# hyx1999/SAM-Decoding

Hardware: AMD Instinct MI355X
Metric: tokens/sec (+ mean accepted tokens), Vicuna-7B bs=1, samd_sam_only draft+verify (higher is better)
Workload: dtype f16

## Files before the change

### sam-decoding_amd/csrc/gemm_kernels.hip

```cpp
#include <hip/hip_runtime.h>
#include <cstdlib>
#include "samd_common.h"

#define LAUNCHCHK() do { hipError_t e_ = hipGetLastError(); if (e_ != hipSuccess) { samd_set_error("kernel launch: %s", hipGetErrorString(e_)); return SAMD_E_HIP; } } while (0)

static int samd_cu_count() { return samd_device_cus(); }

typedef _Float16 half8 __attribute__((ext_vector_type(8)));
typedef __bf16 bf16x8 __attribute__((ext_vector_type(8)));
typedef float floatx4 __attribute__((ext_vector_type(4)));
typedef unsigned u32x4 __attribute__((ext_vector_type(4)));

struct GF16 { typedef _Float16 elem; typedef half8 vec8;
    static __device__ __forceinline__ floatx4 mfma(half8 a, half8 b, floatx4 c) { return __builtin_amdgcn_mfma_f32_16x16x32_f16(a, b, c, 0, 0, 0); } };
struct GBF16 { typedef __bf16 elem; typedef bf16x8 vec8;
    static __device__ __forceinline__ floatx4 mfma(bf16x8 a, bf16x8 b, floatx4 c) { return __builtin_amdgcn_mfma_f32_16x16x32_bf16(a, b, c, 0, 0, 0); } };

#define GEMM_KC 256
#define GEMM_WAVES 8
#define GEMM_COLS (16 * GEMM_WAVES)

typedef __attribute__((address_space(1))) const void *gptr_t;
typedef __attribute__((address_space(3))) void *lptr_t;

#ifdef SAMD_GEMM_ABLATE
__device__ int samd_abl_flag;
#endif

template <typename TT, int RT, int EPI, int DEPTH, bool GM = false>
__global__ __launch_bounds__(64 * GEMM_WAVES, RT >= 3 || DEPTH > 2 ? 2 : GEMM_WAVES / 2) void k_gemm_skinny(const typename TT::elem *__restrict__ A, const typename TT::elem *__restrict__ W,
                                                        float *__restrict__ partial, typename TT::elem *__restrict__ out,
                                                        int K, int N, int n_chunks, int n_splits) {
    typedef typename TT::elem E;
    typedef typename TT::vec8 V8;
    constexpr int R = 16 * RT;
    constexpr int NT = 64 * GEMM_WAVES;
    constexpr int XV = (R * 32) / NT;
    constexpr int NB = DEPTH + 1;
    extern __shared__ __attribute__((aligned(1024))) char gemm_lds[];
    E (*xs)[R][GEMM_KC] = reinterpret_cast<E (*)[R][GEMM_KC]>(gemm_lds);

    const int tid = threadIdx.x, w = tid >> 6, l = tid & 63, n = l & 15, g = l >> 4;
    const int n0 = blockIdx.x * GEMM_COLS + 16 * w;
    const int split = blockIdx.y;
    const int c0 = (int)((long long)split * n_chunks / n_splits), c1 = (int)((long long)(split + 1) * n_chunks / n_splits);
    constexpr size_t WCH = GM ? 8192 : 65536, WU = GM ? 1024 : 8192;
    const int ws = GM ? __builtin_amdgcn_readfirstlane(GEMM_WAVES * (int)blockIdx.x + w) : (int)blockIdx.x;
    const char *wtile = reinterpret_cast<const char *>(W) + (size_t)ws * n_chunks * WCH;
    const uint32_t wlane = (uint32_t)(GM ? l : tid) * 16;
    const uint32_t lds_base = (uint32_t)(uintptr_t)(lptr_t)&xs[0][0][0];

    floatx4 acc[RT];
#pragma unroll
    for (int mt = 0; mt < RT; mt++) acc[mt] = (floatx4){0.f, 0.f, 0.f, 0.f};

    u32x4 wr[DEPTH][4][2];
    auto load_wb = [&](u32x4 (&dst)[4][2], int c, int b) {
        const char *p = wtile + (size_t)c * WCH;
#pragma unroll
        for (int j = 0; j < 2; j++)
            asm volatile("global_load_dwordx4 %0, %1, %2 nt" : "=v"(dst[b][j]) : "v"(wlane), "s"(p + WU * (2 * b + j)) : "memory");
    };
    auto stage_xi = [&](int c, int buf, int i) {
        const int slot = tid + NT * i, row = slot >> 5, pos = slot & 31, unit = pos ^ (row & 15);
        const E *src = A + (size_t)row * K + (size_t)c * GEMM_KC + 8 * unit;
        E *dst = &xs[buf][0][0] + (size_t)(NT * i + 64 * w) * 8;
        __builtin_amdgcn_global_load_lds((gptr_t)src, (lptr_t)dst, 16, 0, 0);
        asm volatile("" ::: "memory");
    };
    auto load_w = [&](u32x4 (&dst)[4][2], int c) {
#pragma unroll
        for (int b = 0; b < 4; b++) load_wb(dst, c, b);
    };
    auto stage_x = [&](int c, int buf) {
#pragma unroll
        for (int i = 0; i < XV; i++) stage_xi(c, buf, i);
    };
    auto landed = [&](int younger_in_flight) {
        if (DEPTH > 2 && younger_in_flight >= 2) asm volatile("s_waitcnt vmcnt(%0)" : : "n"(2 * (8 + XV)) : "memory");
        else if (younger_in_flight >= 1) asm volatile("s_waitcnt vmcnt(%0)" : : "n"(8 + XV) : "memory");
        else asm volatile("s_waitcnt vmcnt(0)" : : : "memory");
        __builtin_amdgcn_s_barrier();
        asm volatile("" ::: "memory");
    };
    auto phase = [&](u32x4 (&cur)[4][2], int c, int buf) {
        landed(c1 - 1 - c);
        const uint32_t xbase = lds_base + (uint32_t)buf * (R * GEMM_KC * 2) + (uint32_t)n * (GEMM_KC * 2);
#pragma unroll
        for (int b = 0; b < 4; b++) {
            const uint32_t u0 = (uint32_t)((8 * b + 2 * g) ^ n) * 16, u1 = (uint32_t)((8 * b + 2 * g + 1) ^ n) * 16;
            const uint32_t a0 = xbase + u0, a1 = xbase + u1;
            u32x4 r[RT][2];
            if constexpr (RT == 1)
                asm volatile("ds_read_b128 %0, %2\n\tds_read_b128 %1, %3\n\ts_waitcnt lgkmcnt(0)" : "=&v"(r[0][0]), "=&v"(r[0][1]) : "v"(a0), "v"(a1));
            else if constexpr (RT == 2)
                asm volatile("ds_read_b128 %0, %4\n\tds_read_b128 %1, %5\n\tds_read_b128 %2, %4 offset:8192\n\tds_read_b128 %3, %5 offset:8192\n\t"
                             "s_waitcnt lgkmcnt(0)" : "=&v"(r[0][0]), "=&v"(r[0][1]), "=&v"(r[1][0]), "=&v"(r[1][1]) : "v"(a0), "v"(a1));
            else if constexpr (RT == 3)
                asm volatile("ds_read_b128 %0, %6\n\tds_read_b128 %1, %7\n\tds_read_b128 %2, %6 offset:8192\n\tds_read_b128 %3, %7 offset:8192\n\t"
                             "ds_read_b128 %4, %6 offset:16384\n\tds_read_b128 %5, %7 offset:16384\n\ts_waitcnt lgkmcnt(0)"
                             : "=&v"(r[0][0]), "=&v"(r[0][1]), "=&v"(r[1][0]), "=&v"(r[1][1]), "=&v"(r[2][0]), "=&v"(r[2][1]) : "v"(a0), "v"(a1));
            else
                asm volatile("ds_read_b128 %0, %8\n\tds_read_b128 %1, %9\n\tds_read_b128 %2, %8 offset:8192\n\tds_read_b128 %3, %9 offset:8192\n\t"
                             "ds_read_b128 %4, %8 offset:16384\n\tds_read_b128 %5, %9 offset:16384\n\tds_read_b128 %6, %8 offset:24576\n\t"
                             "ds_read_b128 %7, %9 offset:24576\n\ts_waitcnt lgkmcnt(0)"
                             : "=&v"(r[0][0]), "=&v"(r[0][1]), "=&v"(r[1][0]), "=&v"(r[1][1]), "=&v"(r[2][0]), "=&v"(r[2][1]), "=&v"(r[3][0]), "=&v"(r[3][1])
                             : "v"(a0), "v"(a1));
#pragma unroll
            for (int mt = 0; mt < RT; mt++) {
                acc[mt] = TT::mfma(__builtin_bit_cast(V8, r[mt][0]), __builtin_bit_cast(V8, cur[b][0]), acc[mt]);
                acc[mt] = TT::mfma(__builtin_bit_cast(V8, r[mt][1]), __builtin_bit_cast(V8, cur[b][1]), acc[mt]);
            }
            if (RT >= 3 && c + DEPTH < c1) {
                load_wb(cur, c + DEPTH, b);
                if (b < XV) stage_xi(c + DEPTH, buf == 0 ? NB - 1 : buf - 1, b);
            }
        }
        if (RT < 3 && c + DEPTH < c1) { load_w(cur, c + DEPTH); stage_x(c + DEPTH, buf == 0 ? NB - 1 : buf - 1); }
    };
    if (c0 < c1) {
#pragma unroll
        for (int d = 0; d < DEPTH; d++)
            if (c0 + d < c1) { load_w(wr[d], c0 + d); stage_x(c0 + d, d); }
        int buf = 0;
        for (int c = c0; c < c1; c += DEPTH) {
#pragma unroll
            for (int d = 0; d < DEPTH; d++)
                if (c + d < c1) { phase(wr[d], c + d, buf); buf = buf == NB - 1 ? 0 : buf + 1; }
        }
    }
    if constexpr (EPI == 1) {
        float *ex = reinterpret_cast<float *>(gemm_lds);
        __syncthreads();
        if (w >= 4) {
#pragma unroll
            for (int mt = 0; mt < RT; mt++)
#pragma unroll
                for (int r = 0; r < 4; r++) ex[(16 * mt + 4 * g + r) * 64 + 16 * (w - 4) + n] = acc[mt][r];
        }
        __syncthreads();
        if (w < 4) {
#pragma unroll
            for (int mt = 0; mt < RT; mt++)
#pragma unroll
                for (int r = 0; r < 4; r++) {
                    const int m = 16 * mt + 4 * g + r;
                    const float gf = (float)(E)acc[mt][r], uf = (float)(E)ex[m * 64 + 16 * w + n];
                    const E sv = (E)(gf / (1.f + __expf(-gf)));
                    out[(size_t)m * (N / 2) + blockIdx.x * 64 + 16 * w + n] = (E)((float)sv * uf);
                }
        }
        return;
    }
#pragma unroll
    for (int mt = 0; mt < RT; mt++) {
#pragma unroll
        for (int r = 0; r < 4; r++) {
            const int m = 16 * mt + 4 * g + r;
            if (out) out[(size_t)m * N + n0 + n] = (E)acc[mt][r];
            else __hip_atomic_store(&partial[((size_t)split * R + m) * N + n0 + n], acc[mt][r], __ATOMIC_RELAXED, __HIP_MEMORY_SCOPE_AGENT);
        }
    }
}

struct NormArgs { const float *ssq; const void *g; int tiles; float inv_hidden; float eps; };

#define NORM_NS 16
template <int NT>
__device__ __forceinline__ void norm_issue(const NormArgs &na, float (&sv)[NORM_NS]) {
    const int tid = threadIdx.x, row = tid & 15, p = tid >> 4;
#pragma unroll
    for (int k = 0; k < NORM_NS; k++) {
        sv[k] = 0.f;
        if ((NT / 16) * k >= na.tiles) continue;
        int t = p + (NT / 16) * k;
        t = t < na.tiles ? t : na.tiles - 1;
        const float *src = na.ssq + (size_t)t * 16 + row;
        asm volatile("global_load_dword %0, %1, off" : "=v"(sv[k]) : "v"(src) : "memory");
    }
}
template <int NT>
__device__ __forceinline__ void norm_finish(const NormArgs &na, float (&sv)[NORM_NS], float *part , float *rs ) {
    const int tid = threadIdx.x, row = tid & 15, p = tid >> 4;
    static_assert(NORM_NS == 16, "");
    asm volatile("" : "+v"(sv[0]), "+v"(sv[1]), "+v"(sv[2]), "+v"(sv[3]), "+v"(sv[4]), "+v"(sv[5]), "+v"(sv[6]), "+v"(sv[7]),
                      "+v"(sv[8]), "+v"(sv[9]), "+v"(sv[10]), "+v"(sv[11]), "+v"(sv[12]), "+v"(sv[13]), "+v"(sv[14]), "+v"(sv[15]) : : "memory");
    float s = 0.f;
#pragma unroll
    for (int k = 0; k < NORM_NS; k++) s += (p + (NT / 16) * k < na.tiles) ? sv[k] : 0.f;
    part[p * 16 + row] = s;
    asm volatile("s_waitcnt lgkmcnt(0)" ::: "memory");
    __builtin_amdgcn_s_barrier();
    asm volatile("" ::: "memory");
    if (tid < 16) {
        float tot = 0.f;
        for (int k = 0; k < NT / 16; k++) tot += part[k * 16 + tid];
        rs[tid] = rsqrtf(tot * na.inv_hidden + na.eps);
    }
    asm volatile("s_waitcnt lgkmcnt(0)" ::: "memory");
    __builtin_amdgcn_s_barrier();
    asm volatile("" ::: "memory");
}

template <typename E>
__device__ __forceinline__ u32x4 norm_scale8(u32x4 xraw, u32x4 graw, float rs) {
    const E *xe = reinterpret_cast<const E *>(&xraw);
    const E *ge = reinterpret_cast<const E *>(&graw);
    u32x4 out;
    E *oe = reinterpret_cast<E *>(&out);
#pragma unroll
    for (int j = 0; j < 8; j++) { const E h = (E)((float)xe[j] * rs); oe[j] = (E)((float)ge[j] * (float)h); }
    return out;
}


template <int DEPTH, int PC>
__device__ __forceinline__ void gemm_wait_younger(int younger) {
    if constexpr (PC == 0) asm volatile("s_waitcnt vmcnt(0)" : : : "memory");
    else {
        if (DEPTH > 3 && younger >= 3) asm volatile("s_waitcnt vmcnt(%0)" : : "n"(3 * PC) : "memory");
        else if (DEPTH > 2 && younger >= 2) asm volatile("s_waitcnt vmcnt(%0)" : : "n"(2 * PC) : "memory");
        else if (younger >= 1) asm volatile("s_waitcnt vmcnt(%0)" : : "n"(PC) : "memory");
        else asm volatile("s_waitcnt vmcnt(0)" : : : "memory");
    }
}

template <typename TT, int RT, int DEPTH, int CG, bool NORM, int AR = 16>
__global__ __launch_bounds__(64 * GEMM_WAVES, RT >= 3 || NORM ? 2 : GEMM_WAVES / 2) void k_gemm_qkv_rope(
        const typename TT::elem *__restrict__ A, const typename TT::elem *__restrict__ W, int K, int n_chunks,
        const float *__restrict__ cs, const int *__restrict__ d_L, const int *__restrict__ d_n,
        typename TT::elem *__restrict__ q_out, typename TT::elem *__restrict__ k_cache, typename TT::elem *__restrict__ v_cache,
        int H, int Hkv, long long max_len, NormArgs na, int v_t) {
    typedef typename TT::elem E;
    typedef typename TT::vec8 V8;
    constexpr int R = 16 * RT;
    constexpr int NT = 64 * GEMM_WAVES;
    constexpr int XV = (R * 32) / NT;
    constexpr int NB = DEPTH + 1;
    constexpr int WL = 4;
    constexpr int TW = 16 * CG, PP = 8 * CG;
    constexpr int CH = CG * 8192;
    extern __shared__ __attribute__((aligned(1024))) char gemm_lds[];
    E (*xs)[R][GEMM_KC] = reinterpret_cast<E (*)[R][GEMM_KC]>(gemm_lds);

    const int tid = threadIdx.x, w = tid >> 6, l = tid & 63, n = l & 15, g = l >> 4;
    const bool streams = CG == 4 || w < 2 * CG;
    static_assert(AR == 16 || (AR == 8 && NORM && RT == 1), "8 activation rows: the norm-fold kernels only");
    const bool stager = AR == 16 || w < GEMM_WAVES / 2;
    const int cg = CG == 4 ? (w & 3) : (streams ? w % CG : 0), kh = CG == 4 ? (w >> 2) : (streams ? w / CG : 0);
    const char *wtile = reinterpret_cast<const char *>(W) + (size_t)blockIdx.x * n_chunks * CH;
    const uint32_t wlane = (uint32_t)(64 * (CG * kh + cg) + l) * 16;
    const uint32_t lds_base = (uint32_t)(uintptr_t)(lptr_t)&xs[0][0][0];
    const int n_rows = d_n[0], L = d_L[0];

    floatx4 acc[RT];
#pragma unroll
    for (int mt = 0; mt < RT; mt++) acc[mt] = (floatx4){0.f, 0.f, 0.f, 0.f};

    u32x4 wr[DEPTH][2][2];
    auto load_wb = [&](u32x4 (&dst)[2][2], int c, int bl) {
        const char *p = wtile + (size_t)c * CH;
#pragma unroll
        for (int j = 0; j < 2; j++)
            asm volatile("global_load_dwordx4 %0, %1, %2 nt" : "=v"(dst[bl][j]) : "v"(wlane), "s"(p + (CH / 4) * (2 * bl + j)) : "memory");
    };
    static_assert(!NORM || RT == 1, "the norm-fold path is built for the 16-row tile");
    constexpr int XL = NORM ? 2 * XV : XV;
    u32x4 xr[NORM ? DEPTH : 1][NORM ? XV : 1], gr[NORM ? DEPTH : 1][NORM ? XV : 1];
    __shared__ float norm_part[NORM ? (NT / 16) * 16 : 1], norm_rs[NORM ? 16 : 1];
    auto stage_xi = [&](int c, int buf, int i, int d) {
        const int slot = tid + NT * i, row = slot >> 5, pos = slot & 31, unit = pos ^ (row & 15);
        const E *src = A + (size_t)row * K + (size_t)c * GEMM_KC + 8 * unit;
        if constexpr (NORM) {
            const E *gsrc = reinterpret_cast<const E *>(na.g) + (size_t)c * GEMM_KC + 8 * unit;
            asm volatile("global_load_dwordx4 %0, %1, off" : "=v"(xr[d][i]) : "v"(src) : "memory");
            asm volatile("global_load_dwordx4 %0, %1, off" : "=v"(gr[d][i]) : "v"(gsrc) : "memory");
        } else {
            E *dst = &xs[buf][0][0] + (size_t)(NT * i + 64 * w) * 8;
            __builtin_amdgcn_global_load_lds((gptr_t)src, (lptr_t)dst, 16, 0, 0);
            asm volatile("" ::: "memory");
        }
    };
    auto issue = [&](u32x4 (&dst)[2][2], int c, int buf, int d) {
        if (streams) { load_wb(dst, c, 0); load_wb(dst, c, 1); }
        if (stager) {
#pragma unroll
            for (int i = 0; i < XV; i++) stage_xi(c, buf, i, d);
        }
    };
    auto scale_to_lds = [&](int buf, int d) {
        if constexpr (NORM) {
            if (!stager) return;
#pragma unroll
            for (int i = 0; i < XV; i++) {
                const int slot = tid + NT * i, row = slot >> 5;
                asm volatile("" : "+v"(xr[d][i]), "+v"(gr[d][i]) : : "memory");
                const u32x4 v = norm_scale8<E>(xr[d][i], gr[d][i], norm_rs[row]);
                *reinterpret_cast<u32x4 *>(&xs[buf][0][0] + (size_t)slot * 8) = v;
            }
        }
    };
    auto landed = [&](int younger, int buf, int d) {
        if (streams) { if (stager) gemm_wait_younger<DEPTH, WL + XL>(younger); else gemm_wait_younger<DEPTH, WL>(younger); }
        else { if (stager) gemm_wait_younger<DEPTH, XL>(younger); else gemm_wait_younger<DEPTH, 0>(younger); }
        if constexpr (NORM) { scale_to_lds(buf, d); asm volatile("s_waitcnt lgkmcnt(0)" ::: "memory"); }
        __builtin_amdgcn_s_barrier();
        asm volatile("" ::: "memory");
    };
    auto phase = [&](u32x4 (&cur)[2][2], int c, int buf, int d) {
        landed(n_chunks - 1 - c, buf, d);
        const uint32_t xbase = lds_base + (uint32_t)buf * (R * GEMM_KC * 2) + (uint32_t)n * (GEMM_KC * 2);
#pragma unroll
        for (int bl = 0; bl < 2; bl++) {
            if (!streams) break;
            const int b = 2 * kh + bl;
            const uint32_t a0 = xbase + (uint32_t)((8 * b + 2 * g) ^ n) * 16, a1 = xbase + (uint32_t)((8 * b + 2 * g + 1) ^ n) * 16;
            u32x4 r[RT][2];
            if constexpr (RT == 1)
                asm volatile("ds_read_b128 %0, %2\n\tds_read_b128 %1, %3\n\ts_waitcnt lgkmcnt(0)" : "=&v"(r[0][0]), "=&v"(r[0][1]) : "v"(a0), "v"(a1));
            else if constexpr (RT == 2)
                asm volatile("ds_read_b128 %0, %4\n\tds_read_b128 %1, %5\n\tds_read_b128 %2, %4 offset:8192\n\tds_read_b128 %3, %5 offset:8192\n\t"
                             "s_waitcnt lgkmcnt(0)" : "=&v"(r[0][0]), "=&v"(r[0][1]), "=&v"(r[1][0]), "=&v"(r[1][1]) : "v"(a0), "v"(a1));
            else if constexpr (RT == 3)
                asm volatile("ds_read_b128 %0, %6\n\tds_read_b128 %1, %7\n\tds_read_b128 %2, %6 offset:8192\n\tds_read_b128 %3, %7 offset:8192\n\t"
                             "ds_read_b128 %4, %6 offset:16384\n\tds_read_b128 %5, %7 offset:16384\n\ts_waitcnt lgkmcnt(0)"
                             : "=&v"(r[0][0]), "=&v"(r[0][1]), "=&v"(r[1][0]), "=&v"(r[1][1]), "=&v"(r[2][0]), "=&v"(r[2][1]) : "v"(a0), "v"(a1));
            else
                asm volatile("ds_read_b128 %0, %8\n\tds_read_b128 %1, %9\n\tds_read_b128 %2, %8 offset:8192\n\tds_read_b128 %3, %9 offset:8192\n\t"
                             "ds_read_b128 %4, %8 offset:16384\n\tds_read_b128 %5, %9 offset:16384\n\tds_read_b128 %6, %8 offset:24576\n\t"
                             "ds_read_b128 %7, %9 offset:24576\n\ts_waitcnt lgkmcnt(0)"
                             : "=&v"(r[0][0]), "=&v"(r[0][1]), "=&v"(r[1][0]), "=&v"(r[1][1]), "=&v"(r[2][0]), "=&v"(r[2][1]), "=&v"(r[3][0]), "=&v"(r[3][1])
                             : "v"(a0), "v"(a1));
#pragma unroll
            for (int mt = 0; mt < RT; mt++) {
                acc[mt] = TT::mfma(__builtin_bit_cast(V8, r[mt][0]), __builtin_bit_cast(V8, cur[bl][0]), acc[mt]);
                acc[mt] = TT::mfma(__builtin_bit_cast(V8, r[mt][1]), __builtin_bit_cast(V8, cur[bl][1]), acc[mt]);
            }
        }
        if (c + DEPTH < n_chunks) issue(cur, c + DEPTH, buf == 0 ? NB - 1 : buf - 1, d);
    };
    float norm_sv[NORM ? NORM_NS : 1];
    if constexpr (NORM) norm_issue<NT>(na, norm_sv);
#pragma unroll
    for (int d = 0; d < DEPTH; d++)
        if (d < n_chunks) issue(wr[d], d, d, d);
    if constexpr (AR == 8) {
        if (!stager) {
#pragma unroll
            for (int bz = 0; bz < NB; bz++) *reinterpret_cast<u32x4 *>(&xs[bz][0][0] + (size_t)tid * 8) = (u32x4){0u, 0u, 0u, 0u};
        }
    }
    if constexpr (NORM) {
        if (n_chunks >= DEPTH) {
            if (streams) { if (stager) asm volatile("s_waitcnt vmcnt(%0)" : : "n"(DEPTH * (WL + XL)) : "memory"); else asm volatile("s_waitcnt vmcnt(%0)" : : "n"(DEPTH * WL) : "memory"); }
            else { if (stager) asm volatile("s_waitcnt vmcnt(%0)" : : "n"(DEPTH * XL) : "memory"); else asm volatile("s_waitcnt vmcnt(0)" : : : "memory"); }
        } else asm volatile("s_waitcnt vmcnt(0)" : : : "memory");
        norm_finish<NT>(na, norm_sv, norm_part, norm_rs);
    }
    {
        int buf = 0;
        for (int c = 0; c < n_chunks; c += DEPTH) {
#pragma unroll
            for (int d = 0; d < DEPTH; d++)
                if (c + d < n_chunks) { phase(wr[d], c + d, buf, d); buf = buf == NB - 1 ? 0 : buf + 1; }
        }
    }
    float *ex = reinterpret_cast<float *>(gemm_lds);
    __syncthreads();
    if (streams) {
#pragma unroll
        for (int mt = 0; mt < RT; mt++)
#pragma unroll
            for (int r = 0; r < 4; r++) ex[(kh * R + 16 * mt + 4 * g + r) * TW + 16 * cg + n] = acc[mt][r];
    }
    __syncthreads();
    const bool vt_tile = v_t && ((PP * (int)blockIdx.x) >> 6) >= H + Hkv;
    for (int i = tid; i < R * PP; i += NT) {
        const int row = vt_tile ? i % R : i / PP, p = vt_tile ? i / R : i % PP;
        if (row >= n_rows || L + row >= max_len) continue;
        const float x1 = (float)(E)(ex[row * TW + p] + ex[(R + row) * TW + p]);
        const float x2 = (float)(E)(ex[row * TW + PP + p] + ex[(R + row) * TW + PP + p]);
        const int pair = PP * (int)blockIdx.x + p, head = pair >> 6, j = pair & 63;
        if (head >= H + Hkv) {
            if (v_t) {
                E *dst = v_cache + (size_t)(head - H - Hkv) * max_len * 128 + L + row;
                dst[(size_t)j * max_len] = (E)x1; dst[(size_t)(j + 64) * max_len] = (E)x2;
                continue;
            }
            E *dst = v_cache + ((size_t)(head - H - Hkv) * max_len + L + row) * 128;
            dst[j] = (E)x1; dst[j + 64] = (E)x2;
            continue;
        }
        const float c = cs[(size_t)row * 128 + j], sn = cs[(size_t)row * 128 + 64 + j];
        const E o1 = (E)(x1 * c - x2 * sn), o2 = (E)(x2 * c + x1 * sn);
        E *dst = head < H ? q_out + ((size_t)row * H + head) * 128 : k_cache + ((size_t)(head - H) * max_len + L + row) * 128;
        dst[j] = o1; dst[j + 64] = o2;
    }
}

template <int CG>
__global__ __launch_bounds__(256) void k_gemm_pack_qkv(const uint4 *__restrict__ W, uint4 *__restrict__ out, int N, int K) {
    const long long u = (long long)blockIdx.x * 256 + threadIdx.x;
    const long long total = (long long)N * K / 8;
    if (u >= total) return;
    constexpr int PP = 8 * CG;
    const int n_chunks = K / GEMM_KC;
    const long long blk = u / (512 * CG);
    const int in = (int)(u % (512 * CG)), jj = in / (128 * CG), x = in % (128 * CG), w = x >> 6, g = (x >> 4) & 3, n = x & 15, cg = w % CG, kh = w / CG;
    const int t = (int)(blk / n_chunks), c = (int)(blk % n_chunks), bl = jj >> 1, j = jj & 1;
    const int q = 16 * cg + n, pair = PP * t + (q < PP ? q : q - PP);
    const long long row = 128LL * (pair >> 6) + (pair & 63) + (q < PP ? 0 : 64), col = 256LL * c + 64 * (2 * kh + bl) + 16 * g + 8 * j;
    out[u] = W[(row * K + col) / 8];
}

static int qkv_tile_groups(int n_heads_total) {
    static const int env = [] { const char *e = getenv("SAMD_QKV_TILE"); return e ? atoi(e) : 0; }();
    const int n_cu = samd_cu_count();
    const int N = n_heads_total * 128;
    if (N % 48 != 0 || env == 64) return 4;
    if (env == 48) return 3;
    const int t48 = N / 48, t64 = N / 64;
    return ((t48 + n_cu - 1) / n_cu) * 48 < ((t64 + n_cu - 1) / n_cu) * 64 ? 3 : 4;
}

template <typename TT, int RT, int DEPTH, bool NORM, int AR = 16>
__global__ __launch_bounds__(64 * GEMM_WAVES, RT >= 3 || DEPTH > 2 ? 2 : GEMM_WAVES / 2) void k_gemm_pairs_silu(const typename TT::elem *__restrict__ A, const typename TT::elem *__restrict__ W,
                                                                                                     typename TT::elem *__restrict__ out, int K, int inter, int n_chunks, int n_pairs, NormArgs na) {
    typedef typename TT::elem E;
    typedef typename TT::vec8 V8;
    constexpr int R = 16 * RT;
    constexpr int NT = 64 * GEMM_WAVES;
    constexpr int XV = (R * 32) / NT;
    constexpr int NB = DEPTH + 1;
    extern __shared__ __attribute__((aligned(1024))) char gemm_lds[];
    E (*xs)[R][GEMM_KC] = reinterpret_cast<E (*)[R][GEMM_KC]>(gemm_lds);

    const int tid = threadIdx.x, w = __builtin_amdgcn_readfirstlane(tid >> 6), l = tid & 63, n = l & 15, g = l >> 4;
#ifdef SAMD_GEMM_ABLATE
    const int abl = samd_abl_flag;
#else
    constexpr int abl = 0;
#endif
    const int p0 = (int)((long long)blockIdx.x * n_pairs / gridDim.x), p1 = (int)((long long)(blockIdx.x + 1) * n_pairs / gridDim.x);
    const bool active = w < 2 * (p1 - p0);
    static_assert(AR == 16 || (AR == 8 && NORM && RT == 1), "8 activation rows: the norm-fold kernels only");
    const bool stager = AR == 16 || w < GEMM_WAVES / 2;
    const int gi = 2 * p0 + w;
    const char *wgrp = reinterpret_cast<const char *>(W) + (size_t)(active ? gi : 0) * n_chunks * 8192;
    const uint32_t wlane = (uint32_t)l * 16;
    const uint32_t lds_base = (uint32_t)(uintptr_t)(lptr_t)&xs[0][0][0];

    floatx4 acc[RT];
#pragma unroll
    for (int mt = 0; mt < RT; mt++) acc[mt] = (floatx4){0.f, 0.f, 0.f, 0.f};
    u32x4 wr[DEPTH][4][2];
    auto load_w = [&](u32x4 (&dst)[4][2], int c) {
        const char *p = wgrp + (size_t)c * 8192;
#pragma unroll
        for (int b = 0; b < 4; b++)
#pragma unroll
            for (int j = 0; j < 2; j++)
                asm volatile("global_load_dwordx4 %0, %1, %2 nt" : "=v"(dst[b][j]) : "v"(wlane), "s"(p + 1024 * (2 * b + j)) : "memory");
    };
    static_assert(!NORM || RT == 1, "the norm-fold path is built for the 16-row tile");
    constexpr int XL = NORM ? 2 * XV : XV;
    u32x4 xr[NORM ? DEPTH : 1][NORM ? XV : 1], gr[NORM ? DEPTH : 1][NORM ? XV : 1];
    __shared__ float norm_part[NORM ? (NT / 16) * 16 : 1], norm_rs[NORM ? 16 : 1];
    auto stage_x = [&](int c, int buf, int d) {
        if (!stager || (abl & 4)) return;
#pragma unroll
        for (int i = 0; i < XV; i++) {
            const int slot = tid + NT * i, row = slot >> 5, pos = slot & 31, unit = pos ^ (row & 15);
            const E *src = A + (size_t)((abl & 8) ? (row & 15) : row) * K + (size_t)c * GEMM_KC + 8 * unit;
            if constexpr (NORM) {
                const E *gsrc = reinterpret_cast<const E *>(na.g) + (size_t)c * GEMM_KC + 8 * unit;
                asm volatile("global_load_dwordx4 %0, %1, off" : "=v"(xr[d][i]) : "v"(src) : "memory");
                asm volatile("global_load_dwordx4 %0, %1, off" : "=v"(gr[d][i]) : "v"(gsrc) : "memory");
            } else {
                E *dst = &xs[buf][0][0] + (size_t)(NT * i + 64 * w) * 8;
                __builtin_amdgcn_global_load_lds((gptr_t)src, (lptr_t)dst, 16, 0, 0);
                asm volatile("" ::: "memory");
            }
        }
    };
    auto landed = [&](int younger, int buf, int d) {
        const bool stg = stager && !(abl & 4);
        if (active) { if (stg) gemm_wait_younger<DEPTH, 8 + XL>(younger); else gemm_wait_younger<DEPTH, 8>(younger); }
        else { if (stg) gemm_wait_younger<DEPTH, XL>(younger); else gemm_wait_younger<DEPTH, 0>(younger); }
        if constexpr (NORM) {
            if (stager) {
#pragma unroll
                for (int i = 0; i < XV; i++) {
                    const int slot = tid + NT * i, row = slot >> 5;
                    asm volatile("" : "+v"(xr[d][i]), "+v"(gr[d][i]) : : "memory");
                    const u32x4 v = norm_scale8<E>(xr[d][i], gr[d][i], norm_rs[row]);
                    *reinterpret_cast<u32x4 *>(&xs[buf][0][0] + (size_t)slot * 8) = v;
                }
            }
            asm volatile("s_waitcnt lgkmcnt(0)" ::: "memory");
        }
        if (!(abl & 1)) __builtin_amdgcn_s_barrier();
        asm volatile("" ::: "memory");
    };
    auto phase = [&](u32x4 (&cur)[4][2], int c, int buf, int d) {
        landed(n_chunks - 1 - c, buf, d);
        if (active && !(abl & 2)) {
            const uint32_t xbase = lds_base + (uint32_t)buf * (R * GEMM_KC * 2) + (uint32_t)n * (GEMM_KC * 2);
#pragma unroll
            for (int b = 0; b < 4; b++) {
                const uint32_t a0 = xbase + (uint32_t)((8 * b + 2 * g) ^ n) * 16, a1 = xbase + (uint32_t)((8 * b + 2 * g + 1) ^ n) * 16;
                u32x4 r[RT][2];
                if constexpr (RT == 1)
                    asm volatile("ds_read_b128 %0, %2\n\tds_read_b128 %1, %3\n\ts_waitcnt lgkmcnt(0)" : "=&v"(r[0][0]), "=&v"(r[0][1]) : "v"(a0), "v"(a1));
                else if constexpr (RT == 2)
                    asm volatile("ds_read_b128 %0, %4\n\tds_read_b128 %1, %5\n\tds_read_b128 %2, %4 offset:8192\n\tds_read_b128 %3, %5 offset:8192\n\t"
                                 "s_waitcnt lgkmcnt(0)" : "=&v"(r[0][0]), "=&v"(r[0][1]), "=&v"(r[1][0]), "=&v"(r[1][1]) : "v"(a0), "v"(a1));
                else if constexpr (RT == 3)
                    asm volatile("ds_read_b128 %0, %6\n\tds_read_b128 %1, %7\n\tds_read_b128 %2, %6 offset:8192\n\tds_read_b128 %3, %7 offset:8192\n\t"
                                 "ds_read_b128 %4, %6 offset:16384\n\tds_read_b128 %5, %7 offset:16384\n\ts_waitcnt lgkmcnt(0)"
                                 : "=&v"(r[0][0]), "=&v"(r[0][1]), "=&v"(r[1][0]), "=&v"(r[1][1]), "=&v"(r[2][0]), "=&v"(r[2][1]) : "v"(a0), "v"(a1));
                else
                    asm volatile("ds_read_b128 %0, %8\n\tds_read_b128 %1, %9\n\tds_read_b128 %2, %8 offset:8192\n\tds_read_b128 %3, %9 offset:8192\n\t"
                                 "ds_read_b128 %4, %8 offset:16384\n\tds_read_b128 %5, %9 offset:16384\n\tds_read_b128 %6, %8 offset:24576\n\t"
                                 "ds_read_b128 %7, %9 offset:24576\n\ts_waitcnt lgkmcnt(0)"
                                 : "=&v"(r[0][0]), "=&v"(r[0][1]), "=&v"(r[1][0]), "=&v"(r[1][1]), "=&v"(r[2][0]), "=&v"(r[2][1]), "=&v"(r[3][0]), "=&v"(r[3][1])
                                 : "v"(a0), "v"(a1));
#pragma unroll
                for (int mt = 0; mt < RT; mt++) {
                    acc[mt] = TT::mfma(__builtin_bit_cast(V8, r[mt][0]), __builtin_bit_cast(V8, cur[b][0]), acc[mt]);
                    acc[mt] = TT::mfma(__builtin_bit_cast(V8, r[mt][1]), __builtin_bit_cast(V8, cur[b][1]), acc[mt]);
                }
            }
        }
        if (c + DEPTH < n_chunks) { if (active) load_w(cur, c + DEPTH); stage_x(c + DEPTH, buf == 0 ? NB - 1 : buf - 1, d); }
    };
    float norm_sv[NORM ? NORM_NS : 1];
    if constexpr (NORM) norm_issue<NT>(na, norm_sv);
#pragma unroll
    for (int d = 0; d < DEPTH; d++)
        if (d < n_chunks) { if (active) load_w(wr[d], d); stage_x(d, d, d); }
    if constexpr (AR == 8) {
        if (!stager) {
#pragma unroll
            for (int bz = 0; bz < NB; bz++) *reinterpret_cast<u32x4 *>(&xs[bz][0][0] + (size_t)tid * 8) = (u32x4){0u, 0u, 0u, 0u};
        }
    }
    if constexpr (NORM) {
        if (n_chunks >= DEPTH) {
            if (active) { if (stager) asm volatile("s_waitcnt vmcnt(%0)" : : "n"(DEPTH * (8 + XL)) : "memory"); else asm volatile("s_waitcnt vmcnt(%0)" : : "n"(DEPTH * 8) : "memory"); }
            else { if (stager) asm volatile("s_waitcnt vmcnt(%0)" : : "n"(DEPTH * XL) : "memory"); else asm volatile("s_waitcnt vmcnt(0)" : : : "memory"); }
        } else asm volatile("s_waitcnt vmcnt(0)" : : : "memory");
        norm_finish<NT>(na, norm_sv, norm_part, norm_rs);
    }
    {
        int buf = 0;
        for (int c = 0; c < n_chunks; c += DEPTH) {
#pragma unroll
            for (int d = 0; d < DEPTH; d++)
                if (c + d < n_chunks) { phase(wr[d], c + d, buf, d); buf = buf == NB - 1 ? 0 : buf + 1; }
        }
    }
    float *ex = reinterpret_cast<float *>(gemm_lds);
    __syncthreads();
    if (active && (w & 1)) {
#pragma unroll
        for (int mt = 0; mt < RT; mt++)
#pragma unroll
            for (int r = 0; r < 4; r++) ex[((w >> 1) * R + 16 * mt + 4 * g + r) * 16 + n] = acc[mt][r];
    }
    __syncthreads();
    if (active && !(w & 1)) {
        const int col = 16 * (p0 + (w >> 1)) + n;
#pragma unroll
        for (int mt = 0; mt < RT; mt++)
#pragma unroll
            for (int r = 0; r < 4; r++) {
                const int m = 16 * mt + 4 * g + r;
                const float gf = (float)(E)acc[mt][r], uf = (float)(E)ex[((w >> 1) * R + m) * 16 + n];
                const E sv = (E)(gf / (1.f + __expf(-gf)));
                out[(size_t)m * inter + col] = (E)((float)sv * uf);
            }
    }
}

template <typename TT, int ROWS, bool EARLY = false>
__global__ __launch_bounds__(64 * GEMM_WAVES, 2) void k_gemm_cs_residual(const typename TT::elem *__restrict__ A, const typename TT::elem *__restrict__ W,
                                                                           typename TT::elem *__restrict__ x, float *__restrict__ ssq, int K, int N, int n_chunks,
                                                                           const int *__restrict__ counter = nullptr, int *__restrict__ epoch = nullptr,
                                                                           int arrivals = 0) {
    typedef typename TT::elem E;
    typedef typename TT::vec8 V8;
    constexpr int CSD = 2;
    extern __shared__ __attribute__((aligned(1024))) char gemm_lds[];
    const int tid = threadIdx.x, w = __builtin_amdgcn_readfirstlane(tid >> 6), l = tid & 63, n = l & 15, g = l >> 4;
    E *xs = reinterpret_cast<E *>(gemm_lds) + (size_t)w * CSD * 16 * GEMM_KC;
    const uint32_t lds_base = (uint32_t)(uintptr_t)(lptr_t)xs;
    const char *wgrp = reinterpret_cast<const char *>(W) + (size_t)blockIdx.x * n_chunks * 8192;
    const uint32_t wlane = (uint32_t)l * 16;

    static_assert(ROWS == 8 || ROWS == 16, "");
    constexpr int AL = ROWS / 2;
    if constexpr (ROWS == 8) {
#pragma unroll
        for (int buf = 0; buf < CSD; buf++)
#pragma unroll
            for (int i = 4; i < 8; i++)
                *reinterpret_cast<u32x4 *>(xs + (size_t)buf * 16 * GEMM_KC + (size_t)(64 * i + l) * 8) = (u32x4){0u, 0u, 0u, 0u};
        asm volatile("s_waitcnt lgkmcnt(0)" ::: "memory");
    }
    floatx4 acc = (floatx4){0.f, 0.f, 0.f, 0.f};
    u32x4 wr[CSD][4][2];
    auto issue_w = [&](u32x4 (&dst)[4][2], int c) {
        const char *p = wgrp + (size_t)c * 8192;
#pragma unroll
        for (int b = 0; b < 4; b++)
#pragma unroll
            for (int j = 0; j < 2; j++)
                asm volatile("global_load_dwordx4 %0, %1, %2 nt" : "=v"(dst[b][j]) : "v"(wlane), "s"(p + 1024 * (2 * b + j)) : "memory");
    };
    auto issue_a = [&](int c, int buf) {
#pragma unroll
        for (int i = 0; i < AL; i++) {
            const int slot = l + 64 * i, row = slot >> 5, pos = slot & 31, unit = pos ^ (row & 15);
            const E *src = A + (size_t)row * K + (size_t)c * GEMM_KC + 8 * unit;
            E *dst_l = xs + (size_t)buf * 16 * GEMM_KC + (size_t)(64 * i) * 8;
            __builtin_amdgcn_global_load_lds((gptr_t)src, (lptr_t)dst_l, 16, 0, 0);
            asm volatile("" ::: "memory");
        }
    };
    auto issue = [&](u32x4 (&dst)[4][2], int c, int buf) { issue_w(dst, c); issue_a(c, buf); };
    auto phase = [&](u32x4 (&cur)[4][2], int c, int buf, bool more) {
        if (more) { if constexpr (EARLY) asm volatile("s_waitcnt vmcnt(%0)" : : "n"(AL) : "memory"); else asm volatile("s_waitcnt vmcnt(%0)" : : "n"(8 + AL) : "memory"); }
        else asm volatile("s_waitcnt vmcnt(0)" ::: "memory");
        const uint32_t xbase = lds_base + (uint32_t)buf * (16 * GEMM_KC * 2) + (uint32_t)n * (GEMM_KC * 2);
#pragma unroll
        for (int b = 0; b < 4; b++) {
            const uint32_t a0 = xbase + (uint32_t)((8 * b + 2 * g) ^ n) * 16, a1 = xbase + (uint32_t)((8 * b + 2 * g + 1) ^ n) * 16;
            u32x4 r0, r1;
            asm volatile("ds_read_b128 %0, %2\n\tds_read_b128 %1, %3\n\ts_waitcnt lgkmcnt(0)" : "=&v"(r0), "=&v"(r1) : "v"(a0), "v"(a1));
            acc = TT::mfma(__builtin_bit_cast(V8, r0), __builtin_bit_cast(V8, cur[b][0]), acc);
            acc = TT::mfma(__builtin_bit_cast(V8, r1), __builtin_bit_cast(V8, cur[b][1]), acc);
        }
    };
    const int mine = (n_chunks - w + GEMM_WAVES - 1) / GEMM_WAVES;
    if constexpr (EARLY) {
        if (mine > 0) issue_w(wr[0], w);
        if (mine > 1) issue_w(wr[1], w + GEMM_WAVES);
        __shared__ int my_epoch;
        if (tid == 0) {
            const int e = epoch[blockIdx.x];
            const int target = (e + 1) * arrivals;
            for (int spin = 0; spin < (1 << 22); spin++) {
                if (__hip_atomic_load(counter, __ATOMIC_RELAXED, __HIP_MEMORY_SCOPE_AGENT) >= target) break;
                __builtin_amdgcn_s_sleep(4);
            }
            my_epoch = e;
        }
        __syncthreads();
        __builtin_amdgcn_fence(__ATOMIC_ACQUIRE, "agent");
        if (mine > 0) issue_a(w, 0);
        if (mine > 1) issue_a(w + GEMM_WAVES, 1);
        if (mine > 0) phase(wr[0], w, 0, mine > 1);
        if (mine > 1) phase(wr[1], w + GEMM_WAVES, 1, false);
        if (tid == 0) epoch[blockIdx.x] = my_epoch + 1;
    } else {
        if (mine > 0) issue(wr[0], w, 0);
        if (mine > 1) issue(wr[1], w + GEMM_WAVES, 1);
        for (int i = 0; i < mine; i += 2) {
            phase(wr[0], w + GEMM_WAVES * i, 0, i + 1 < mine);
            if (i + 2 < mine) issue(wr[0], w + GEMM_WAVES * (i + 2), 0);
            if (i + 1 < mine) {
                phase(wr[1], w + GEMM_WAVES * (i + 1), 1, i + 2 < mine);
                if (i + 3 < mine) issue(wr[1], w + GEMM_WAVES * (i + 3), 1);
            }
        }
    }
    __syncthreads();
    float *ex = reinterpret_cast<float *>(gemm_lds);
#pragma unroll
    for (int r = 0; r < 4; r++) ex[(w * 16 + 4 * g + r) * 16 + n] = acc[r];
    __syncthreads();
    if (tid < 16 * ROWS) {
        const int row = tid >> 4, col = tid & 15;
        float sum = 0.f;
#pragma unroll
        for (int k = 0; k < GEMM_WAVES; k++) sum += ex[(k * 16 + row) * 16 + col];
        E *xp = x + (size_t)row * N + 16 * blockIdx.x + col;
        const E o = (E)sum;
        const E y = (E)((float)*xp + (float)o);
        *xp = y;
        float q = (float)y * (float)y;
        q += __shfl_xor(q, 1); q += __shfl_xor(q, 2); q += __shfl_xor(q, 4); q += __shfl_xor(q, 8);
        if (col == 0) ssq[(size_t)blockIdx.x * 16 + row] = q;
    }
}

__global__ __launch_bounds__(256) void k_gemm_pack_groups(const uint4 *__restrict__ W, uint4 *__restrict__ out, int N, int K) {
    const long long u = (long long)blockIdx.x * 256 + threadIdx.x;
    const long long total = (long long)N * K / 8;
    if (u >= total) return;
    const int n_chunks = K / GEMM_KC;
    const long long blk = u >> 9;
    const int in = (int)(u & 511), jj = in >> 6, lane = in & 63, g = lane >> 4, n = lane & 15, b = jj >> 1, j = jj & 1;
    const long long gi = blk / n_chunks; const int c = (int)(blk % n_chunks);
    const long long row = 16 * gi + n, col = 256LL * c + 64 * b + 16 * g + 8 * j;
    out[u] = W[(row * K + col) / 8];
}

__global__ __launch_bounds__(256) void k_gemm_pack(const uint4 *__restrict__ W, uint4 *__restrict__ out, int N, int K) {
    const long long u = (long long)blockIdx.x * 256 + threadIdx.x;
    const long long total = (long long)N * K / 8;
    if (u >= total) return;
    const int n_chunks = K / GEMM_KC;
    const long long blk = u >> 12;
    const int in = (int)(u & 4095), jj = in >> 9, tid = in & 511, w = tid >> 6, g = (tid >> 4) & 3, n = tid & 15;
    const int t = (int)(blk / n_chunks), c = (int)(blk % n_chunks), b = jj >> 1, j = jj & 1;
    const long long row = 128LL * t + 16 * w + n, col = 256LL * c + 64 * b + 16 * g + 8 * j;
    out[u] = W[(row * K + col) / 8];
}

template <typename TT, int RT, int EPI, int DEPTH, bool GM = false>
static hipError_t gemm_launch(dim3 grid, hipStream_t st, const void *A, const void *W, float *partial, void *out, int K, int N, int chunks, int splits) {
    constexpr int lds = (DEPTH + 1) * 16 * RT * GEMM_KC * 2;
    if constexpr (lds > 65536) {
        static unsigned long long done = 0ull;
        const hipError_t attr = samd_reserve_lds((const void *)k_gemm_skinny<TT, RT, EPI, DEPTH, GM>, lds, &done);
        if (attr != hipSuccess) return attr;
    }
    hipLaunchKernelGGL((k_gemm_skinny<TT, RT, EPI, DEPTH, GM>), grid, dim3(64 * GEMM_WAVES), lds, st, (const typename TT::elem *)A, (const typename TT::elem *)W, partial,
                       (typename TT::elem *)out, K, N, chunks, splits);
    return hipSuccess;
}

template <int EPI, bool GM = false>
static hipError_t gemm_dispatch(int dtype, int rows_pad, dim3 grid, hipStream_t st, const void *A, const void *W, float *partial, void *out, int K, int N, int chunks,
                                int splits) {
#define GO(TT, RT, D) return gemm_launch<TT, RT, EPI, D, GM>(grid, st, A, W, partial, out, K, N, chunks, splits)
#define ROWS(TT) do { if (rows_pad == 16) GO(TT, 1, 2); else if (rows_pad == 32) GO(TT, 2, 2); else if (rows_pad == 48) GO(TT, 3, 2); else GO(TT, 4, 2); } while (0)
    if (dtype == SAMD_F16) ROWS(GF16); else ROWS(GBF16);
#undef ROWS
#undef GO
}

template <typename TT, int RT, int DEPTH, int CG, bool NORM = false, int AR = 16>
static hipError_t qkv_rope_launch(hipStream_t st, const void *A, const void *W, int K, int tiles, const float *cs, const int *d_L, const int *d_n, void *q, void *k, void *v,
                                  int H, int Hkv, long long max_len, int v_t, NormArgs na = NormArgs{nullptr, nullptr, 0, 0.f, 0.f}) {
    constexpr int lds_a = (DEPTH + 1) * 16 * RT * GEMM_KC * 2, lds_e = 2 * 16 * RT * 16 * CG * 4, lds = lds_a > lds_e ? lds_a : lds_e;
    if constexpr (lds > 60000) {
        static unsigned long long done = 0ull;
        const hipError_t attr = samd_reserve_lds((const void *)k_gemm_qkv_rope<TT, RT, DEPTH, CG, NORM, AR>, lds + 4096, &done);
        if (attr != hipSuccess) return attr;
    }
    hipLaunchKernelGGL((k_gemm_qkv_rope<TT, RT, DEPTH, CG, NORM, AR>), dim3(tiles), dim3(64 * GEMM_WAVES), lds, st, (const typename TT::elem *)A, (const typename TT::elem *)W, K, K / GEMM_KC,
                       cs, d_L, d_n, (typename TT::elem *)q, (typename TT::elem *)k, (typename TT::elem *)v, H, Hkv, max_len, na, v_t);
    return hipSuccess;
}

template <typename TT, int RT, int DEPTH, bool NORM = false, int AR = 16>
static hipError_t pairs_silu_launch(hipStream_t st, int grid, const void *A, const void *W, void *out, int K, int inter, int n_pairs,
                                    NormArgs na = NormArgs{nullptr, nullptr, 0, 0.f, 0.f}) {
    constexpr int lds_a = (DEPTH + 1) * 16 * RT * GEMM_KC * 2, lds_e = 4 * 16 * RT * 16 * 4, lds = lds_a > lds_e ? lds_a : lds_e;
    if constexpr (lds > 60000) {
        static unsigned long long done = 0ull;
        const hipError_t attr = samd_reserve_lds((const void *)k_gemm_pairs_silu<TT, RT, DEPTH, NORM, AR>, lds + 4096, &done);
        if (attr != hipSuccess) return attr;
    }
    hipLaunchKernelGGL((k_gemm_pairs_silu<TT, RT, DEPTH, NORM, AR>), dim3(grid), dim3(64 * GEMM_WAVES), lds, st, (const typename TT::elem *)A, (const typename TT::elem *)W,
                       (typename TT::elem *)out, K, inter, K / GEMM_KC, n_pairs, na);
    return hipSuccess;
}

extern "C" {

int samd_gemm_splits(int32_t N, int32_t K, int32_t rows_pad) {
    static const int env_cap = [] { const char *e = getenv("SAMD_GEMM_SPLIT_CAP"); const int v = e ? atoi(e) : 8; return v < 1 ? 1 : (v > 8 ? 8 : v); }();
    static const int env_fixed = [] { const char *e = getenv("SAMD_GEMM_SPLITS"); const int v = e ? atoi(e) : 0; return v < 0 ? 0 : (v > 8 ? 8 : v); }();
    const int cols = N / GEMM_COLS, chunks = K / GEMM_KC;
    (void)rows_pad;
    if (env_fixed) return env_fixed > chunks ? (chunks < 1 ? 1 : chunks) : env_fixed;
    int s = 256 / (cols > 0 ? cols : 1);
    if (s > env_cap) s = env_cap;
    if (s > chunks) s = chunks;
    return s < 1 ? 1 : s;
}

int64_t samd_gemm_workspace(int32_t rows_pad, int32_t N, int32_t splits) { return (int64_t)splits * rows_pad * N * 4; }

int samd_gemm_skinny_silu(const void *d_A, const void *d_W, int32_t rows_pad, int32_t N, int32_t K, void *d_out, int32_t dtype, void *stream) {
    if (!d_A || !d_W || !d_out || (rows_pad != 16 && rows_pad != 32 && rows_pad != 48 && rows_pad != 64) || N < GEMM_COLS || N % GEMM_COLS != 0 || K < GEMM_KC ||
        K % GEMM_KC != 0 || (dtype != SAMD_F16 && dtype != SAMD_BF16)) {
        samd_set_error("samd_gemm_skinny_silu: unsupported shape (rows 16/32/48/64, N %% 128 == 0, K %% 256 == 0) or null pointer"); return SAMD_E_INVALID;
    }
    const hipError_t e = gemm_dispatch<1>(dtype, rows_pad, dim3(N / GEMM_COLS, 1), (hipStream_t)stream, d_A, d_W, nullptr, d_out, K, N, K / GEMM_KC, 1);
    if (e != hipSuccess) { samd_set_error("samd_gemm_skinny_silu: %s", hipGetErrorString(e)); return SAMD_E_HIP; }
    LAUNCHCHK();
    return SAMD_OK;
}

int samd_gemm_pack_weights(const void *d_W, void *d_packed, int32_t N, int32_t K, void *stream) {
    if (!d_W || !d_packed || d_W == d_packed || N < GEMM_COLS || N % GEMM_COLS != 0 || K < GEMM_KC || K % GEMM_KC != 0) {
        samd_set_error("samd_gemm_pack_weights: needs N %% 128 == 0, K %% 256 == 0 and distinct buffers"); return SAMD_E_INVALID;
    }
    const long long units = (long long)N * K / 8;
    hipLaunchKernelGGL(k_gemm_pack, dim3((unsigned)((units + 255) / 256)), dim3(256), 0, (hipStream_t)stream, (const uint4 *)d_W, (uint4 *)d_packed, N, K);
    LAUNCHCHK();
    return SAMD_OK;
}

int samd_gemm_pack_groups(const void *d_W, void *d_packed, int32_t N, int32_t K, void *stream) {
    if (!d_W || !d_packed || d_W == d_packed || N < 16 || N % 16 != 0 || K < GEMM_KC || K % GEMM_KC != 0) {
        samd_set_error("samd_gemm_pack_groups: needs N %% 16 == 0, K %% 256 == 0 and distinct buffers"); return SAMD_E_INVALID;
    }
    const long long units = (long long)N * K / 8;
    hipLaunchKernelGGL(k_gemm_pack_groups, dim3((unsigned)((units + 255) / 256)), dim3(256), 0, (hipStream_t)stream, (const uint4 *)d_W, (uint4 *)d_packed, N, K);
    LAUNCHCHK();
    return SAMD_OK;
}

int samd_gemm_pairs_silu_norm(const void *d_x, const float *d_ssq, const void *d_norm_weight, float eps, const void *d_Wg, int32_t rows_pad, int32_t inter, int32_t K,
                              void *d_out, int32_t dtype, void *stream) {
    if (!d_x || !d_ssq || !d_norm_weight || !d_Wg || !d_out || (rows_pad != 16 && rows_pad != 8) || inter < 16 || inter % 16 != 0 || K < GEMM_KC || K % GEMM_KC != 0 ||
        K / 16 > 32 * NORM_NS || (dtype != SAMD_F16 && dtype != SAMD_BF16)) {
        samd_set_error("samd_gemm_pairs_silu_norm: unsupported shape (8 or 16 rows, inter %% 16 == 0, K %% 256 == 0, K <= 8192, f16/bf16) or null pointer"); return SAMD_E_INVALID;
    }
    const int n_cu = samd_cu_count();
    const int n_pairs = inter / 16;
    int grid = n_pairs < n_cu ? n_pairs : n_cu;
    while ((n_pairs + grid - 1) / grid > 4) grid += n_cu;
    const NormArgs na{d_ssq, d_norm_weight, K / 16, 1.f / (float)K, eps};
    hipStream_t st = (hipStream_t)stream;
    const hipError_t e = rows_pad == 8
        ? (dtype == SAMD_F16 ? pairs_silu_launch<GF16, 1, 3, true, 8>(st, grid, d_x, d_Wg, d_out, K, inter, n_pairs, na)
                             : pairs_silu_launch<GBF16, 1, 3, true, 8>(st, grid, d_x, d_Wg, d_out, K, inter, n_pairs, na))
        : (dtype == SAMD_F16 ? pairs_silu_launch<GF16, 1, 3, true>(st, grid, d_x, d_Wg, d_out, K, inter, n_pairs, na)
                             : pairs_silu_launch<GBF16, 1, 3, true>(st, grid, d_x, d_Wg, d_out, K, inter, n_pairs, na));
    if (e != hipSuccess) { samd_set_error("samd_gemm_pairs_silu_norm: %s", hipGetErrorString(e)); return SAMD_E_HIP; }
    LAUNCHCHK();
    return SAMD_OK;
}

int samd_gemm_cs_residual(const void *d_A, const void *d_Wg, int32_t rows_pad, int32_t N, int32_t K, void *d_x, float *d_ssq, int32_t dtype, void *stream) {
    if (!d_A || !d_Wg || !d_x || !d_ssq || (rows_pad != 16 && rows_pad != 8) || N < 16 || N % 16 != 0 || K < GEMM_KC || K % GEMM_KC != 0 || (dtype != SAMD_F16 && dtype != SAMD_BF16)) {
        samd_set_error("samd_gemm_cs_residual: unsupported shape (8 or 16 rows, N %% 16 == 0, K %% 256 == 0, f16/bf16) or null pointer"); return SAMD_E_INVALID;
    }
    constexpr int lds = GEMM_WAVES * 2 * 16 * GEMM_KC * 2;
    hipStream_t st = (hipStream_t)stream;
    hipError_t e = hipSuccess;
#define GO(TT, ROWS, ET) do { static unsigned long long done = 0ull; \
        e = samd_reserve_lds((const void *)k_gemm_cs_residual<TT, ROWS>, lds, &done); \
        if (e == hipSuccess) hipLaunchKernelGGL((k_gemm_cs_residual<TT, ROWS>), dim3(N / 16), dim3(64 * GEMM_WAVES), lds, st, (const ET *)d_A, (const ET *)d_Wg, (ET *)d_x, d_ssq, K, N, K / GEMM_KC, (const int *)nullptr, (int *)nullptr, 0); } while (0)
    if (dtype == SAMD_F16) { if (rows_pad == 8) GO(GF16, 8, _Float16); else GO(GF16, 16, _Float16); }
    else { if (rows_pad == 8) GO(GBF16, 8, __bf16); else GO(GBF16, 16, __bf16); }
#undef GO
    if (e != hipSuccess) { samd_set_error("samd_gemm_cs_residual: %s", hipGetErrorString(e)); return SAMD_E_HIP; }
    LAUNCHCHK();
    return SAMD_OK;
}

int samd_gemm_cs_residual_early(const void *d_A, const void *d_Wg, int32_t N, int32_t K, void *d_x, float *d_ssq, int32_t dtype, const int32_t *d_counter,
                                int32_t *d_epoch, int32_t arrivals, void *stream) {
    if (!d_A || !d_Wg || !d_x || !d_ssq || !d_counter || !d_epoch || arrivals < 1 || N < 16 || N % 16 != 0 || K != 2 * GEMM_WAVES * GEMM_KC ||
        (dtype != SAMD_F16 && dtype != SAMD_BF16)) {
        samd_set_error("samd_gemm_cs_residual_early: unsupported shape (K must be 4096, N %% 16 == 0, f16/bf16) or null pointer"); return SAMD_E_INVALID;
    }
    constexpr int lds = GEMM_WAVES * 2 * 16 * GEMM_KC * 2;
    hipStream_t st = (hipStream_t)stream;
    hipError_t e = hipSuccess;
    if (dtype == SAMD_F16) {
        static unsigned long long done = 0ull;
        e = samd_reserve_lds((const void *)k_gemm_cs_residual<GF16, 8, true>, lds, &done);
        if (e == hipSuccess) hipLaunchKernelGGL((k_gemm_cs_residual<GF16, 8, true>), dim3(N / 16), dim3(64 * GEMM_WAVES), lds, st, (const _Float16 *)d_A, (const _Float16 *)d_Wg,
                                                (_Float16 *)d_x, d_ssq, K, N, K / GEMM_KC, d_counter, d_epoch, arrivals);
    } else {
        static unsigned long long done = 0ull;
        e = samd_reserve_lds((const void *)k_gemm_cs_residual<GBF16, 8, true>, lds, &done);
        if (e == hipSuccess) hipLaunchKernelGGL((k_gemm_cs_residual<GBF16, 8, true>), dim3(N / 16), dim3(64 * GEMM_WAVES), lds, st, (const __bf16 *)d_A, (const __bf16 *)d_Wg,
                                                (__bf16 *)d_x, d_ssq, K, N, K / GEMM_KC, d_counter, d_epoch, arrivals);
    }
    if (e != hipSuccess) { samd_set_error("samd_gemm_cs_residual_early: %s", hipGetErrorString(e)); return SAMD_E_HIP; }
    LAUNCHCHK();
    return SAMD_OK;
}

int samd_gemm_pairs_silu(const void *d_A, const void *d_Wg, int32_t rows_pad, int32_t inter, int32_t K, void *d_out, int32_t dtype, void *stream) {
    if (!d_A || !d_Wg || !d_out || (rows_pad != 16 && rows_pad != 32 && rows_pad != 48 && rows_pad != 64) || inter < 16 || inter % 16 != 0 || K < GEMM_KC ||
        K % GEMM_KC != 0 || (dtype != SAMD_F16 && dtype != SAMD_BF16)) {
        samd_set_error("samd_gemm_pairs_silu: unsupported shape (rows 16/32/48/64, inter %% 16 == 0, K %% 256 == 0, f16/bf16) or null pointer"); return SAMD_E_INVALID;
    }
    const int n_cu = samd_cu_count();
    const int n_pairs = inter / 16;
    int grid = n_pairs < n_cu ? n_pairs : n_cu;
    while ((n_pairs + grid - 1) / grid > 4) grid += n_cu;
    hipStream_t st = (hipStream_t)stream;
    hipError_t e;
    static const int depth_env = [] { const char *e = getenv("SAMD_PAIRS_DEPTH"); return e ? atoi(e) : 0; }();
#ifdef SAMD_GEMM_ABLATE
    static const int abl_set = [] { const char *e = getenv("SAMD_GEMM_ABL"); const int v = e ? atoi(e) : 0; return hipMemcpyToSymbol(HIP_SYMBOL(samd_abl_flag), &v, 4) == hipSuccess ? 1 : -1; }();
    (void)abl_set;
#endif
#define ARGS st, grid, d_A, d_Wg, d_out, K, inter, n_pairs
#define GO(TT) (rows_pad == 16 ? (depth_env == 2 ? pairs_silu_launch<TT, 1, 2>(ARGS) : depth_env == 4 ? pairs_silu_launch<TT, 1, 4>(ARGS) : pairs_silu_launch<TT, 1, 3>(ARGS)) \
                : rows_pad == 32 ? (depth_env == 2 ? pairs_silu_launch<TT, 2, 2>(ARGS) : pairs_silu_launch<TT, 2, 3>(ARGS)) \
                : rows_pad == 48 ? pairs_silu_launch<TT, 3, 2>(ARGS) : pairs_silu_launch<TT, 4, 2>(ARGS))
    e = dtype == SAMD_F16 ? GO(GF16) : GO(GBF16);
#undef GO
#undef ARGS
    if (e != hipSuccess) { samd_set_error("samd_gemm_pairs_silu: %s", hipGetErrorString(e)); return SAMD_E_HIP; }
    LAUNCHCHK();
    return SAMD_OK;
}

int samd_gemm_pack_qkv64(const void *d_W, void *d_packed, int32_t n_heads_total, int32_t K, void *stream) {
    if (!d_W || !d_packed || d_W == d_packed || n_heads_total < 1 || K < GEMM_KC || K % GEMM_KC != 0) {
        samd_set_error("samd_gemm_pack_qkv64: needs K %% 256 == 0, whole 128-column heads and distinct buffers"); return SAMD_E_INVALID;
    }
    const long long units = (long long)n_heads_total * 128 * K / 8;
    if (qkv_tile_groups(n_heads_total) == 3)
        hipLaunchKernelGGL(k_gemm_pack_qkv<3>, dim3((unsigned)((units + 255) / 256)), dim3(256), 0, (hipStream_t)stream, (const uint4 *)d_W, (uint4 *)d_packed, n_heads_total * 128, K);
    else
        hipLaunchKernelGGL(k_gemm_pack_qkv<4>, dim3((unsigned)((units + 255) / 256)), dim3(256), 0, (hipStream_t)stream, (const uint4 *)d_W, (uint4 *)d_packed, n_heads_total * 128, K);
    LAUNCHCHK();
    return SAMD_OK;
}

static int gemm_qkv_rope_impl(const void *d_A, const void *d_W64, int32_t rows_pad, int32_t K, const float *d_cs, const int32_t *d_cache_length, const int32_t *d_n,
                              void *d_q_out, void *d_k_cache, void *d_v_cache, int32_t n_heads, int32_t n_kv_heads, int32_t head_dim, int64_t max_len,
                              int32_t dtype, void *stream, int v_t) {
    if (!d_A || !d_W64 || !d_cs || !d_cache_length || !d_n || !d_q_out || !d_k_cache || !d_v_cache || head_dim != 128 || n_heads < 1 || n_kv_heads < 1 ||
        (rows_pad != 16 && rows_pad != 32 && rows_pad != 48 && rows_pad != 64) || K < GEMM_KC || K % GEMM_KC != 0 || (dtype != SAMD_F16 && dtype != SAMD_BF16)) {
        samd_set_error("samd_gemm_qkv_rope: unsupported shape (rows 16/32/48/64, head_dim 128, K %% 256 == 0, f16/bf16) or null pointer"); return SAMD_E_INVALID;
    }
    static const int depth_env = [] { const char *e = getenv("SAMD_QKV_DEPTH"); return e ? atoi(e) : 0; }();
    const int groups = qkv_tile_groups(n_heads + 2 * n_kv_heads);
    const int tiles = (n_heads + 2 * n_kv_heads) * 128 / (16 * groups);
    hipStream_t st = (hipStream_t)stream;
    hipError_t e = hipSuccess;
#define GO(TT, RT, D, CG) e = qkv_rope_launch<TT, RT, D, CG>(st, d_A, d_W64, K, tiles, d_cs, d_cache_length, d_n, d_q_out, d_k_cache, d_v_cache, n_heads, n_kv_heads, (long long)max_len, v_t)
#define ROWS(TT, CG) do { if (rows_pad == 16) { if (depth_env == 2) GO(TT, 1, 2, CG); else if (depth_env == 3) GO(TT, 1, 3, CG); else GO(TT, 1, 4, CG); } \
                          else if (rows_pad == 32) { if (depth_env == 2) GO(TT, 2, 2, CG); else GO(TT, 2, 4, CG); } \
                          else if (rows_pad == 48) GO(TT, 3, 3, CG); else GO(TT, 4, 3, CG); } while (0)
    if (groups == 3) { if (dtype == SAMD_F16) ROWS(GF16, 3); else ROWS(GBF16, 3); }
    else { if (dtype == SAMD_F16) ROWS(GF16, 4); else ROWS(GBF16, 4); }
#undef ROWS
#undef GO
    if (e != hipSuccess) { samd_set_error("samd_gemm_qkv_rope: %s", hipGetErrorString(e)); return SAMD_E_HIP; }
    LAUNCHCHK();
    return SAMD_OK;
}

int samd_gemm_qkv_rope(const void *d_A, const void *d_W64, int32_t rows_pad, int32_t K, const float *d_cs, const int32_t *d_cache_length, const int32_t *d_n,
                       void *d_q_out, void *d_k_cache, void *d_v_cache, int32_t n_heads, int32_t n_kv_heads, int32_t head_dim, int64_t max_len,
                       int32_t dtype, void *stream) {
    return gemm_qkv_rope_impl(d_A, d_W64, rows_pad, K, d_cs, d_cache_length, d_n, d_q_out, d_k_cache, d_v_cache, n_heads, n_kv_heads, head_dim, max_len, dtype, stream, 0);
}

int samd_gemm_qkv_rope_vt(const void *d_A, const void *d_W64, int32_t rows_pad, int32_t K, const float *d_cs, const int32_t *d_cache_length, const int32_t *d_n,
                          void *d_q_out, void *d_k_cache, void *d_vt_cache, int32_t n_heads, int32_t n_kv_heads, int32_t head_dim, int64_t max_len,
                          int32_t dtype, void *stream) {
    return gemm_qkv_rope_impl(d_A, d_W64, rows_pad, K, d_cs, d_cache_length, d_n, d_q_out, d_k_cache, d_vt_cache, n_heads, n_kv_heads, head_dim, max_len, dtype, stream, 1);
}

static int gemm_qkv_rope_norm_impl(const void *d_x, const float *d_ssq, const void *d_norm_weight, float eps, const void *d_W64, int32_t rows_pad, int32_t K,
                                   const float *d_cs, const int32_t *d_cache_length, const int32_t *d_n, void *d_q_out, void *d_k_cache, void *d_v_cache,
                                   int32_t n_heads, int32_t n_kv_heads, int32_t head_dim, int64_t max_len, int32_t dtype, void *stream, int v_t) {
    if (!d_x || !d_ssq || !d_norm_weight || !d_W64 || !d_cs || !d_cache_length || !d_n || !d_q_out || !d_k_cache || !d_v_cache || head_dim != 128 || n_heads < 1 ||
        n_kv_heads < 1 || (rows_pad != 16 && rows_pad != 8) || K < GEMM_KC || K % GEMM_KC != 0 || K / 16 > 32 * NORM_NS || (dtype != SAMD_F16 && dtype != SAMD_BF16)) {
        samd_set_error("samd_gemm_qkv_rope_norm: unsupported shape (8 or 16 rows, head_dim 128, K %% 256 == 0, K <= 8192, f16/bf16) or null pointer"); return SAMD_E_INVALID;
    }
    const int groups = qkv_tile_groups(n_heads + 2 * n_kv_heads);
    const int tiles = (n_heads + 2 * n_kv_heads) * 128 / (16 * groups);
    const NormArgs na{d_ssq, d_norm_weight, K / 16, 1.f / (float)K, eps};
    hipStream_t st = (hipStream_t)stream;
    hipError_t e = hipSuccess;
#define GO(TT, CG, AR) e = qkv_rope_launch<TT, 1, 4, CG, true, AR>(st, d_x, d_W64, K, tiles, d_cs, d_cache_length, d_n, d_q_out, d_k_cache, d_v_cache, n_heads, n_kv_heads, (long long)max_len, v_t, na)
    if (rows_pad == 8) {
        if (groups == 3) { if (dtype == SAMD_F16) GO(GF16, 3, 8); else GO(GBF16, 3, 8); }
        else { if (dtype == SAMD_F16) GO(GF16, 4, 8); else GO(GBF16, 4, 8); }
    } else {
        if (groups == 3) { if (dtype == SAMD_F16) GO(GF16, 3, 16); else GO(GBF16, 3, 16); }
        else { if (dtype == SAMD_F16) GO(GF16, 4, 16); else GO(GBF16, 4, 16); }
    }
#undef GO
    if (e != hipSuccess) { samd_set_error("samd_gemm_qkv_rope_norm: %s", hipGetErrorString(e)); return SAMD_E_HIP; }
    LAUNCHCHK();
    return SAMD_OK;
}

int samd_gemm_qkv_rope_norm(const void *d_x, const float *d_ssq, const void *d_norm_weight, float eps, const void *d_W64, int32_t rows_pad, int32_t K,
                            const float *d_cs, const int32_t *d_cache_length, const int32_t *d_n, void *d_q_out, void *d_k_cache, void *d_v_cache,
                            int32_t n_heads, int32_t n_kv_heads, int32_t head_dim, int64_t max_len, int32_t dtype, void *stream) {
    return gemm_qkv_rope_norm_impl(d_x, d_ssq, d_norm_weight, eps, d_W64, rows_pad, K, d_cs, d_cache_length, d_n, d_q_out, d_k_cache, d_v_cache, n_heads, n_kv_heads, head_dim,
                                   max_len, dtype, stream, 0);
}

int samd_gemm_qkv_rope_norm_vt(const void *d_x, const float *d_ssq, const void *d_norm_weight, float eps, const void *d_W64, int32_t rows_pad, int32_t K,
                               const float *d_cs, const int32_t *d_cache_length, const int32_t *d_n, void *d_q_out, void *d_k_cache, void *d_vt_cache,
                               int32_t n_heads, int32_t n_kv_heads, int32_t head_dim, int64_t max_len, int32_t dtype, void *stream) {
    return gemm_qkv_rope_norm_impl(d_x, d_ssq, d_norm_weight, eps, d_W64, rows_pad, K, d_cs, d_cache_length, d_n, d_q_out, d_k_cache, d_vt_cache, n_heads, n_kv_heads, head_dim,
                                   max_len, dtype, stream, 1);
}

int samd_gemm_skinny(const void *d_A, const void *d_W, int32_t rows_pad, int32_t N, int32_t K, int32_t splits, float *d_partial,
                     void *d_out, int32_t dtype, void *stream) {
    if (!d_A || !d_W || (rows_pad != 16 && rows_pad != 32 && rows_pad != 48 && rows_pad != 64) || N < GEMM_COLS || N % GEMM_COLS != 0 || K < GEMM_KC ||
        K % GEMM_KC != 0 || splits < 1 || splits > K / GEMM_KC || (splits == 1 ? !d_out : !d_partial) || (dtype != SAMD_F16 && dtype != SAMD_BF16)) {
        samd_set_error("samd_gemm_skinny: unsupported shape (rows 16/32/48/64, N %% 128 == 0, K %% 256 == 0) or null pointer"); return SAMD_E_INVALID;
    }
    const hipError_t e = gemm_dispatch<0>(dtype, rows_pad, dim3(N / GEMM_COLS, splits), (hipStream_t)stream, d_A, d_W, d_partial, splits == 1 ? d_out : nullptr, K, N,
                                          K / GEMM_KC, splits);
    if (e != hipSuccess) { samd_set_error("samd_gemm_skinny: %s", hipGetErrorString(e)); return SAMD_E_HIP; }
    LAUNCHCHK();
    return SAMD_OK;
}

int samd_gemm_skinny_groups(const void *d_A, const void *d_Wg, int32_t rows_pad, int32_t N, int32_t K, int32_t splits, float *d_partial,
                            void *d_out, int32_t dtype, void *stream) {
    if (!d_A || !d_Wg || (rows_pad != 16 && rows_pad != 32 && rows_pad != 48 && rows_pad != 64) || N < GEMM_COLS || N % GEMM_COLS != 0 || K < GEMM_KC ||
        K % GEMM_KC != 0 || splits < 1 || splits > K / GEMM_KC || (splits == 1 ? !d_out : !d_partial) || (dtype != SAMD_F16 && dtype != SAMD_BF16)) {
        samd_set_error("samd_gemm_skinny_groups: unsupported shape (rows 16/32/48/64, N %% 128 == 0, K %% 256 == 0) or null pointer"); return SAMD_E_INVALID;
    }
    const hipError_t e = gemm_dispatch<0, true>(dtype, rows_pad, dim3(N / GEMM_COLS, splits), (hipStream_t)stream, d_A, d_Wg, d_partial, splits == 1 ? d_out : nullptr, K, N,
                                                K / GEMM_KC, splits);
    if (e != hipSuccess) { samd_set_error("samd_gemm_skinny_groups: %s", hipGetErrorString(e)); return SAMD_E_HIP; }
    LAUNCHCHK();
    return SAMD_OK;
}

}

template <typename TT> struct F8Widen;
template <> struct F8Widen<GF16> {
    static __device__ __forceinline__ half8 cvt(unsigned w0, unsigned w1) {
        const auto a = __builtin_amdgcn_cvt_scalef32_pk_f16_fp8(w0, 1.0f, false), b = __builtin_amdgcn_cvt_scalef32_pk_f16_fp8(w0, 1.0f, true);
        const auto c = __builtin_amdgcn_cvt_scalef32_pk_f16_fp8(w1, 1.0f, false), d = __builtin_amdgcn_cvt_scalef32_pk_f16_fp8(w1, 1.0f, true);
        return __builtin_bit_cast(half8, (u32x4){__builtin_bit_cast(unsigned, a), __builtin_bit_cast(unsigned, b), __builtin_bit_cast(unsigned, c), __builtin_bit_cast(unsigned, d)});
    }
};
template <> struct F8Widen<GBF16> {
    static __device__ __forceinline__ bf16x8 cvt(unsigned w0, unsigned w1) {
        const auto a = __builtin_amdgcn_cvt_scalef32_pk_bf16_fp8(w0, 1.0f, false), b = __builtin_amdgcn_cvt_scalef32_pk_bf16_fp8(w0, 1.0f, true);
        const auto c = __builtin_amdgcn_cvt_scalef32_pk_bf16_fp8(w1, 1.0f, false), d = __builtin_amdgcn_cvt_scalef32_pk_bf16_fp8(w1, 1.0f, true);
        return __builtin_bit_cast(bf16x8, (u32x4){__builtin_bit_cast(unsigned, a), __builtin_bit_cast(unsigned, b), __builtin_bit_cast(unsigned, c), __builtin_bit_cast(unsigned, d)});
    }
};

template <typename TT, int RT, int DEPTH>
__global__ __launch_bounds__(64 * GEMM_WAVES, 2) void k_gemm_skinny_f8(const typename TT::elem *__restrict__ A, const unsigned char *__restrict__ W8,
                                                                     const float *__restrict__ scale, float *__restrict__ partial,
                                                                     typename TT::elem *__restrict__ out, int K, int N, int n_chunks, int n_splits) {
    typedef typename TT::elem E;
    constexpr int R = 16 * RT;
    constexpr int NT = 64 * GEMM_WAVES;
    constexpr int XV = (R * 32) / NT;
    constexpr int NB = DEPTH + 1;
    constexpr int PC = 4 + XV;
    constexpr size_t WCH = 32768, WU = 8192;
    extern __shared__ __attribute__((aligned(1024))) char gemm_lds[];
    E (*xs)[R][GEMM_KC] = reinterpret_cast<E (*)[R][GEMM_KC]>(gemm_lds);

    const int tid = threadIdx.x, w = tid >> 6, l = tid & 63, n = l & 15, g = l >> 4;
    const int n0 = blockIdx.x * GEMM_COLS + 16 * w;
    const int split = blockIdx.y;
    const int c0 = (int)((long long)split * n_chunks / n_splits), c1 = (int)((long long)(split + 1) * n_chunks / n_splits);
    const char *wtile = reinterpret_cast<const char *>(W8) + (size_t)blockIdx.x * n_chunks * WCH;
    const uint32_t wlane = (uint32_t)tid * 16;
    const uint32_t lds_base = (uint32_t)(uintptr_t)(lptr_t)&xs[0][0][0];
    const float sc = scale[n0 + n];

    floatx4 acc[RT];
#pragma unroll
    for (int mt = 0; mt < RT; mt++) acc[mt] = (floatx4){0.f, 0.f, 0.f, 0.f};

    u32x4 wr[DEPTH][4];
    auto load_wb = [&](u32x4 (&dst)[4], int c, int b) {
        const char *p = wtile + (size_t)c * WCH;
        asm volatile("global_load_dwordx4 %0, %1, %2 nt" : "=v"(dst[b]) : "v"(wlane), "s"(p + WU * b) : "memory");
    };
    auto stage_xi = [&](int c, int buf, int i) {
        const int slot = tid + NT * i, row = slot >> 5, pos = slot & 31, unit = pos ^ (row & 15);
        const E *src = A + (size_t)row * K + (size_t)c * GEMM_KC + 8 * unit;
        E *dst = &xs[buf][0][0] + (size_t)(NT * i + 64 * w) * 8;
        __builtin_amdgcn_global_load_lds((gptr_t)src, (lptr_t)dst, 16, 0, 0);
        asm volatile("" ::: "memory");
    };
    auto load_w = [&](u32x4 (&dst)[4], int c) {
#pragma unroll
        for (int b = 0; b < 4; b++) load_wb(dst, c, b);
    };
    auto stage_x = [&](int c, int buf) {
#pragma unroll
        for (int i = 0; i < XV; i++) stage_xi(c, buf, i);
    };
    auto phase = [&](u32x4 (&cur)[4], int c, int buf) {
        gemm_wait_younger<DEPTH, PC>(c1 - 1 - c);
        __builtin_amdgcn_s_barrier();
        asm volatile("" ::: "memory");
        const uint32_t xbase = lds_base + (uint32_t)buf * (R * GEMM_KC * 2) + (uint32_t)n * (GEMM_KC * 2);
#pragma unroll
        for (int b = 0; b < 4; b++) {
            const uint32_t a0 = xbase + (uint32_t)((8 * b + 2 * g) ^ n) * 16, a1 = xbase + (uint32_t)((8 * b + 2 * g + 1) ^ n) * 16;
            u32x4 r[RT][2];
            if constexpr (RT == 1)
                asm volatile("ds_read_b128 %0, %2\n\tds_read_b128 %1, %3\n\ts_waitcnt lgkmcnt(0)" : "=&v"(r[0][0]), "=&v"(r[0][1]) : "v"(a0), "v"(a1));
            else if constexpr (RT == 2)
                asm volatile("ds_read_b128 %0, %4\n\tds_read_b128 %1, %5\n\tds_read_b128 %2, %4 offset:8192\n\tds_read_b128 %3, %5 offset:8192\n\t"
                             "s_waitcnt lgkmcnt(0)" : "=&v"(r[0][0]), "=&v"(r[0][1]), "=&v"(r[1][0]), "=&v"(r[1][1]) : "v"(a0), "v"(a1));
            else if constexpr (RT == 3)
                asm volatile("ds_read_b128 %0, %6\n\tds_read_b128 %1, %7\n\tds_read_b128 %2, %6 offset:8192\n\tds_read_b128 %3, %7 offset:8192\n\t"
                             "ds_read_b128 %4, %6 offset:16384\n\tds_read_b128 %5, %7 offset:16384\n\ts_waitcnt lgkmcnt(0)"
                             : "=&v"(r[0][0]), "=&v"(r[0][1]), "=&v"(r[1][0]), "=&v"(r[1][1]), "=&v"(r[2][0]), "=&v"(r[2][1]) : "v"(a0), "v"(a1));
            else
                asm volatile("ds_read_b128 %0, %8\n\tds_read_b128 %1, %9\n\tds_read_b128 %2, %8 offset:8192\n\tds_read_b128 %3, %9 offset:8192\n\t"
                             "ds_read_b128 %4, %8 offset:16384\n\tds_read_b128 %5, %9 offset:16384\n\tds_read_b128 %6, %8 offset:24576\n\t"
                             "ds_read_b128 %7, %9 offset:24576\n\ts_waitcnt lgkmcnt(0)"
                             : "=&v"(r[0][0]), "=&v"(r[0][1]), "=&v"(r[1][0]), "=&v"(r[1][1]), "=&v"(r[2][0]), "=&v"(r[2][1]), "=&v"(r[3][0]), "=&v"(r[3][1])
                             : "v"(a0), "v"(a1));
            asm volatile("" : "+v"(cur[b]) : : "memory");
            const auto lo = F8Widen<TT>::cvt(cur[b][0], cur[b][1]), hi = F8Widen<TT>::cvt(cur[b][2], cur[b][3]);
#pragma unroll
            for (int mt = 0; mt < RT; mt++) {
                acc[mt] = TT::mfma(__builtin_bit_cast(typename TT::vec8, r[mt][0]), lo, acc[mt]);
                acc[mt] = TT::mfma(__builtin_bit_cast(typename TT::vec8, r[mt][1]), hi, acc[mt]);
            }
            if (RT >= 3 && c + DEPTH < c1) {
                load_wb(cur, c + DEPTH, b);
                if (b < XV) stage_xi(c + DEPTH, buf == 0 ? NB - 1 : buf - 1, b);
            }
        }
        if (RT < 3 && c + DEPTH < c1) { load_w(cur, c + DEPTH); stage_x(c + DEPTH, buf == 0 ? NB - 1 : buf - 1); }
    };
    if (c0 < c1) {
#pragma unroll
        for (int d = 0; d < DEPTH; d++)
            if (c0 + d < c1) { load_w(wr[d], c0 + d); stage_x(c0 + d, d); }
        int buf = 0;
        for (int c = c0; c < c1; c += DEPTH) {
#pragma unroll
            for (int d = 0; d < DEPTH; d++)
                if (c + d < c1) { phase(wr[d], c + d, buf); buf = buf == NB - 1 ? 0 : buf + 1; }
        }
    }
#pragma unroll
    for (int mt = 0; mt < RT; mt++) {
#pragma unroll
        for (int r = 0; r < 4; r++) {
            const int m = 16 * mt + 4 * g + r;
            const float v = acc[mt][r] * sc;
            if (out) out[(size_t)m * N + n0 + n] = (E)v;
            else __hip_atomic_store(&partial[((size_t)split * R + m) * N + n0 + n], v, __ATOMIC_RELAXED, __HIP_MEMORY_SCOPE_AGENT);
        }
    }
}

__global__ __launch_bounds__(256) void k_gemm_pack_f8(const uint4 *__restrict__ W8, uint4 *__restrict__ out, int N, int K) {
    const long long u = (long long)blockIdx.x * 256 + threadIdx.x;
    const long long total = (long long)N * K / 16;
    if (u >= total) return;
    const int n_chunks = K / GEMM_KC;
    const long long blk = u >> 11;
    const int in = (int)(u & 2047), b = in >> 9, tid = in & 511, w = tid >> 6, g = (tid >> 4) & 3, n = tid & 15;
    const int t = (int)(blk / n_chunks), c = (int)(blk % n_chunks);
    const long long row = 128LL * t + 16 * w + n, col = 256LL * c + 64 * b + 16 * g;
    out[u] = W8[(row * K + col) / 16];
}

template <typename TT, int RT, int DEPTH>
static hipError_t gemm_f8_launch(dim3 grid, hipStream_t st, const void *A, const void *W8, const float *scale, float *partial, void *out, int K, int N,
                                 int splits) {
    constexpr int lds = (DEPTH + 1) * 16 * RT * GEMM_KC * 2;
    if constexpr (lds > 65536) {
        static unsigned long long done = 0ull;
        const hipError_t attr = samd_reserve_lds((const void *)k_gemm_skinny_f8<TT, RT, DEPTH>, lds, &done);
        if (attr != hipSuccess) return attr;
    }
    hipLaunchKernelGGL((k_gemm_skinny_f8<TT, RT, DEPTH>), grid, dim3(64 * GEMM_WAVES), lds, st, (const typename TT::elem *)A, (const unsigned char *)W8, scale,
                       partial, (typename TT::elem *)out, K, N, K / GEMM_KC, splits);
    return hipSuccess;
}

extern "C" {

int samd_gemm_pack_f8(const void *d_W8, void *d_out, int32_t N, int32_t K, void *stream) {
    if (!d_W8 || !d_out || d_W8 == d_out || N < GEMM_COLS || N % GEMM_COLS != 0 || K < GEMM_KC || K % GEMM_KC != 0) {
        samd_set_error("samd_gemm_pack_f8: needs N %% 128 == 0, K %% 256 == 0 and distinct buffers"); return SAMD_E_INVALID;
    }
    const long long units = (long long)N * K / 16;
    hipLaunchKernelGGL(k_gemm_pack_f8, dim3((unsigned)((units + 255) / 256)), dim3(256), 0, (hipStream_t)stream, (const uint4 *)d_W8, (uint4 *)d_out, N, K);
    LAUNCHCHK();
    return SAMD_OK;
}

int samd_gemm_skinny_f8(const void *d_A, const void *d_W8p, const float *d_scale, int32_t rows_pad, int32_t N, int32_t K, int32_t splits, float *d_partial,
                        void *d_out, int32_t dtype, void *stream) {
    if (!d_A || !d_W8p || !d_scale || (rows_pad != 16 && rows_pad != 32 && rows_pad != 48 && rows_pad != 64) || N < GEMM_COLS || N % GEMM_COLS != 0 ||
        K < GEMM_KC || K % GEMM_KC != 0 || splits < 1 || splits > K / GEMM_KC || (splits == 1 ? !d_out : !d_partial) || (dtype != SAMD_F16 && dtype != SAMD_BF16)) {
        samd_set_error("samd_gemm_skinny_f8: unsupported shape (rows 16/32/48/64, N %% 128 == 0, K %% 256 == 0) or null pointer"); return SAMD_E_INVALID;
    }
    const dim3 grid(N / GEMM_COLS, splits);
    const hipStream_t st = (hipStream_t)stream;
    float *part = splits == 1 ? nullptr : d_partial;
    void *out = splits == 1 ? d_out : nullptr;
#define GO(TT, RT, D) e = gemm_f8_launch<TT, RT, D>(grid, st, d_A, d_W8p, d_scale, part, out, K, N, splits)
#define ROWS(TT) do { if (rows_pad == 16) GO(TT, 1, 4); else if (rows_pad == 32) GO(TT, 2, 4); else if (rows_pad == 48) GO(TT, 3, 4); else GO(TT, 4, 3); } while (0)
    hipError_t e;
    if (dtype == SAMD_F16) ROWS(GF16); else ROWS(GBF16);
#undef ROWS
#undef GO
    if (e != hipSuccess) { samd_set_error("samd_gemm_skinny_f8: %s", hipGetErrorString(e)); return SAMD_E_HIP; }
    LAUNCHCHK();
    return SAMD_OK;
}

}

template <typename TT> struct F4Widen;
template <> struct F4Widen<GF16> {
    static __device__ __forceinline__ half8 cvt(unsigned w, float s) {
        const auto a = __builtin_amdgcn_cvt_scalef32_pk_f16_fp4(w, s, 0), b = __builtin_amdgcn_cvt_scalef32_pk_f16_fp4(w, s, 1);
        const auto c = __builtin_amdgcn_cvt_scalef32_pk_f16_fp4(w, s, 2), d = __builtin_amdgcn_cvt_scalef32_pk_f16_fp4(w, s, 3);
        return __builtin_bit_cast(half8, (u32x4){__builtin_bit_cast(unsigned, a), __builtin_bit_cast(unsigned, b), __builtin_bit_cast(unsigned, c), __builtin_bit_cast(unsigned, d)});
    }
};
template <> struct F4Widen<GBF16> {
    static __device__ __forceinline__ bf16x8 cvt(unsigned w, float s) {
        const auto a = __builtin_amdgcn_cvt_scalef32_pk_bf16_fp4(w, s, 0), b = __builtin_amdgcn_cvt_scalef32_pk_bf16_fp4(w, s, 1);
        const auto c = __builtin_amdgcn_cvt_scalef32_pk_bf16_fp4(w, s, 2), d = __builtin_amdgcn_cvt_scalef32_pk_bf16_fp4(w, s, 3);
        return __builtin_bit_cast(bf16x8, (u32x4){__builtin_bit_cast(unsigned, a), __builtin_bit_cast(unsigned, b), __builtin_bit_cast(unsigned, c), __builtin_bit_cast(unsigned, d)});
    }
};

template <int DEPTH, int PC>
__device__ __forceinline__ void gemm_wait_younger_deep(int younger) {
    static_assert(DEPTH <= 8 && (DEPTH - 1) * PC <= 63, "vmcnt is a 6-bit counter");
#define SAMD_WAIT_IF(i) if (DEPTH > i && younger >= i) { asm volatile("s_waitcnt vmcnt(%0)" : : "n"(DEPTH > i ? i * PC : 0) : "memory"); return; }
    SAMD_WAIT_IF(7) SAMD_WAIT_IF(6) SAMD_WAIT_IF(5) SAMD_WAIT_IF(4) SAMD_WAIT_IF(3) SAMD_WAIT_IF(2) SAMD_WAIT_IF(1)
#undef SAMD_WAIT_IF
    asm volatile("s_waitcnt vmcnt(0)" : : : "memory");
}

template <int RT>
__device__ __forceinline__ void gemm_f4_read_a(u32x4 (&r)[RT][2], uint32_t a0, uint32_t a1) {
    if constexpr (RT == 1)
        asm volatile("ds_read_b128 %0, %2\n\tds_read_b128 %1, %3\n\ts_waitcnt lgkmcnt(0)" : "=&v"(r[0][0]), "=&v"(r[0][1]) : "v"(a0), "v"(a1));
    else if constexpr (RT == 2)
        asm volatile("ds_read_b128 %0, %4\n\tds_read_b128 %1, %5\n\tds_read_b128 %2, %4 offset:8192\n\tds_read_b128 %3, %5 offset:8192\n\t"
                     "s_waitcnt lgkmcnt(0)" : "=&v"(r[0][0]), "=&v"(r[0][1]), "=&v"(r[1][0]), "=&v"(r[1][1]) : "v"(a0), "v"(a1));
    else if constexpr (RT == 3)
        asm volatile("ds_read_b128 %0, %6\n\tds_read_b128 %1, %7\n\tds_read_b128 %2, %6 offset:8192\n\tds_read_b128 %3, %7 offset:8192\n\t"
                     "ds_read_b128 %4, %6 offset:16384\n\tds_read_b128 %5, %7 offset:16384\n\ts_waitcnt lgkmcnt(0)"
                     : "=&v"(r[0][0]), "=&v"(r[0][1]), "=&v"(r[1][0]), "=&v"(r[1][1]), "=&v"(r[2][0]), "=&v"(r[2][1]) : "v"(a0), "v"(a1));
    else
        asm volatile("ds_read_b128 %0, %8\n\tds_read_b128 %1, %9\n\tds_read_b128 %2, %8 offset:8192\n\tds_read_b128 %3, %9 offset:8192\n\t"
                     "ds_read_b128 %4, %8 offset:16384\n\tds_read_b128 %5, %9 offset:16384\n\tds_read_b128 %6, %8 offset:24576\n\t"
                     "ds_read_b128 %7, %9 offset:24576\n\ts_waitcnt lgkmcnt(0)"
                     : "=&v"(r[0][0]), "=&v"(r[0][1]), "=&v"(r[1][0]), "=&v"(r[1][1]), "=&v"(r[2][0]), "=&v"(r[2][1]), "=&v"(r[3][0]), "=&v"(r[3][1])
                     : "v"(a0), "v"(a1));
}

template <typename TT, int RT, int DEPTH>
__global__ __launch_bounds__(64 * GEMM_WAVES, 2) void k_gemm_skinny_f4(const typename TT::elem *__restrict__ A, const unsigned char *__restrict__ W4,
                                                                     float *__restrict__ partial, typename TT::elem *__restrict__ out, int K, int N,
                                                                     int n_chunks, int n_splits) {
    typedef typename TT::elem E;
    constexpr int R = 16 * RT;
    constexpr int NT = 64 * GEMM_WAVES;
    constexpr int XV = (R * 32) / NT;
    constexpr int NB = DEPTH + 1;
    constexpr int PC = 3 + XV;
    constexpr size_t WCH = 17408, WU = 8192, WS = 16384;
    extern __shared__ __attribute__((aligned(1024))) char gemm_lds[];
    E (*xs)[R][GEMM_KC] = reinterpret_cast<E (*)[R][GEMM_KC]>(gemm_lds);

    const int tid = threadIdx.x, w = tid >> 6, l = tid & 63, n = l & 15, g = l >> 4;
    const int n0 = blockIdx.x * GEMM_COLS + 16 * w;
    const int split = blockIdx.y;
    const int c0 = (int)((long long)split * n_chunks / n_splits), c1 = (int)((long long)(split + 1) * n_chunks / n_splits);
    const char *wtile = reinterpret_cast<const char *>(W4) + (size_t)blockIdx.x * n_chunks * WCH;
    const uint32_t wlane = (uint32_t)tid * 16, slane = (uint32_t)tid * 2;
    const uint32_t lds_base = (uint32_t)(uintptr_t)(lptr_t)&xs[0][0][0];

    floatx4 acc[RT];
#pragma unroll
    for (int mt = 0; mt < RT; mt++) acc[mt] = (floatx4){0.f, 0.f, 0.f, 0.f};

// ... 1261 lines not shown
```

### sam-decoding_amd/samd_hip/llama.py

```python
import ctypes as C
import math
import os

import torch

from . import (F16, BF16, MAX_DRAFT, TILE_ROWS, QkvEpilogue, SamdError, Session, Warm, _ptr, check, current_stream, lib, require_gpu,
               torch_dtype_code)
from . import fp8 as F8
from . import mxfp4 as MX
from . import int4 as I4
from . import moe as MOE


def _env_weight_format(weight_format):
    return weight_format if weight_format is not None else (os.environ.get("SAMD_WEIGHT_FORMAT") or None)


def _weight_format(weight_format, weights, dtype):
    has_f8 = any(l[k].dtype == torch.float8_e4m3fn for l in weights["layers"] for k in F8.PROJECTIONS if k in l)
    has_i4 = any(k + "_z" in l for l in weights["layers"] for k in I4.PROJECTIONS)
    has_f4 = any(_is_f4_tensor(l[k]) and k + "_z" not in l for l in weights["layers"] for k in MX.PROJECTIONS if k in l)
    names = {torch.float16: ("fp16", "float16", "half"), torch.bfloat16: ("bf16", "bfloat16")}.get(dtype, ())
    if weight_format is None:
        fmt = "fp8" if has_f8 else ("mxfp4" if has_f4 else ("int4g128" if has_i4 else None))
    elif weight_format in ("fp8", "mxfp4", "int4g128"):
        fmt = weight_format
    elif weight_format == dtype or (isinstance(weight_format, str) and weight_format.lower() in names):
        fmt = None
    else:
        hint = " (the AWQ / GPTQ format is spelled 'int4g128': 4-bit codes in groups of 128, the only group size the kernel has)" \
            if weight_format == "int4" else ""
        raise SamdError(f"weight_format {weight_format!r}: expected None, 'fp8', 'mxfp4', 'int4g128' or the model dtype ({dtype}){hint}")
    if has_f8 and fmt != "fp8":
        raise SamdError(f"the weights carry float8_e4m3fn projections; weight_format {weight_format!r} would need them dequantised (pass None or 'fp8')")
    if has_f4 and fmt != "mxfp4":
        raise SamdError(f"the weights carry MXFP4 projections; weight_format {weight_format!r} would need them dequantised (pass None or 'mxfp4')")
    if has_i4 and fmt != "int4g128":
        raise SamdError(f"the weights carry INT4 (AWQ / GPTQ) projections; weight_format {weight_format!r} would need them dequantised (pass None or 'int4g128')")
    return fmt


def _is_f4_tensor(t):
    return t.dtype == torch.uint8 or MX.is_fp4_dtype(t.dtype)


def _cfg_get(cfg, name, default=None):
    if isinstance(cfg, dict):
        return cfg.get(name, default)
    return getattr(cfg, name, default)


class LlamaShape:

    def __init__(self, cfg, qkv_bias=None, qk_norm=None):
        self.hidden = int(_cfg_get(cfg, "hidden_size"))
        self.inter = int(_cfg_get(cfg, "intermediate_size"))
        self.layers = int(_cfg_get(cfg, "num_hidden_layers"))
        self.heads = int(_cfg_get(cfg, "num_attention_heads"))
        kv = _cfg_get(cfg, "num_key_value_heads")
        self.kv_heads = int(kv) if kv is not None else self.heads
        hd = _cfg_get(cfg, "head_dim")
        self.head_dim = int(hd) if hd else self.hidden // self.heads
        self.vocab = int(_cfg_get(cfg, "vocab_size"))
        self.eps = float(_cfg_get(cfg, "rms_norm_eps", 1e-6))
        self.max_pos = int(_cfg_get(cfg, "max_position_embeddings", 2048))
        rp = _cfg_get(cfg, "rope_parameters") or _cfg_get(cfg, "rope_scaling") or {}
        theta = _cfg_get(cfg, "rope_theta")
        if theta is None and isinstance(rp, dict):
            theta = rp.get("rope_theta")
        self.rope_theta = float(theta if theta is not None else 10000.0)
        self.rope_scaling = dict(rp) if isinstance(rp, dict) else {}
        if self.head_dim != 128:
            raise SamdError("the gfx950 tree-attention kernel is specialised for head_dim 128 (Vicuna-7B / Llama-3-8B)")
        self.model_type = str(_cfg_get(cfg, "model_type", None) or "llama")
        layer_types = _cfg_get(cfg, "layer_types", None) or ()
        if _cfg_get(cfg, "use_sliding_window", False) or any(t != "full_attention" for t in layer_types):
            raise SamdError("sliding-window attention layers are not supported (use_sliding_window / layer_types)")
        if _cfg_get(cfg, "attention_bias", False):
            raise SamdError("attention_bias=True puts a bias on o_proj, which the runner does not support (q|k|v biases alone are)")
        if _cfg_get(cfg, "mlp_bias", False):
            raise SamdError("MLP projection biases (mlp_bias=True) are not supported")
        self.qkv_bias = (self.model_type == "qwen2") if qkv_bias is None else bool(qkv_bias)
        self.qk_norm = (self.model_type in ("qwen3", "qwen3_moe")) if qk_norm is None else bool(qk_norm)
        self.n_experts = self.top_k = self.moe_inter = 0
        self.norm_topk = False
        self.sparse = [False] * self.layers
        if self.model_type == "qwen3_moe":
            self.n_experts = int(_cfg_get(cfg, "num_experts", 0) or 0)
            self.top_k = int(_cfg_get(cfg, "num_experts_per_tok", 0) or 0)
            self.moe_inter = int(_cfg_get(cfg, "moe_intermediate_size", 0) or 0)
            self.norm_topk = bool(_cfg_get(cfg, "norm_topk_prob", False))
            self.sparse = MOE.sparse_layer_map(self.layers, self.n_experts, _cfg_get(cfg, "mlp_only_layers"), _cfg_get(cfg, "decoder_sparse_step", 1))
        self.moe = any(self.sparse)
        if self.moe:
            MOE.check_shape(self.hidden, self.moe_inter, self.n_experts, self.top_k)

    def inv_freq(self):
        d = self.head_dim
        inv = 1.0 / (self.rope_theta ** (torch.arange(0, d, 2, dtype=torch.float64) / d))
        rs = self.rope_scaling
        kind = rs.get("rope_type", rs.get("type", "default")) if rs else "default"
        if kind == "llama3":
            factor, lo, hi = rs["factor"], rs["low_freq_factor"], rs["high_freq_factor"]
            old = rs["original_max_position_embeddings"]
            wavelen = 2 * math.pi / inv
            scaled = torch.where(wavelen > old / lo, inv / factor, inv)
            smooth = (old / wavelen - lo) / (hi - lo)
            mid = (1 - smooth) * inv / factor + smooth * inv
            is_mid = (wavelen <= old / lo) & (wavelen >= old / hi)
            inv = torch.where(is_mid, mid, scaled)
        elif kind == "linear":
            inv = inv / rs["factor"]
        elif kind not in ("default", None):
            raise SamdError(f"unsupported rope scaling '{kind}'")
        return inv


class LlamaRunner:

    BUCKETS = (1, 8, 16, 32, 48, 64, 128)

    def __init__(self, shape, weights, max_cache_len, dtype=torch.float16, device="cuda", kv=None, native_gemm=True, packed_lm_head=None,
                 attention=None, weight_format=None, draft_head=False, expert_format=MOE.AUTO):
        sparse_l = [l for l in weights["layers"] if "experts_gu" in l]
        experts_i4 = [any(k in l for k in ("experts_gu_z", "experts_gu_s", "experts_down_z", "experts_down_s")) for l in sparse_l]
        experts4 = [not i4e and (MOE.is_4bit(l["experts_gu"]) or MOE.is_4bit(l["experts_down"])) for l, i4e in zip(sparse_l, experts_i4)]
        self.expert_format = MOE.resolve_expert_format(expert_format, any(experts4), shape.moe,
                                                       carries_int4=any(experts_i4))
        if shape.moe:
            MOE.reject_unsupported(_weight_format(weight_format, weights, dtype), native_gemm, draft_head)
        if any(experts4):
            if not all(experts4):
                raise SamdError(f"a mix of 4-bit and model-dtype sparse layers ({sum(experts4)} of {len(experts4)} carry MXFP4 experts): "
                                "the runner takes the experts of all sparse layers in one format")
            for i, l in enumerate(weights["layers"]):
                if "experts_gu" in l:
                    MOE.check_quantised_experts(l["experts_gu"], l.get("experts_gu_scale"), l["experts_down"], l.get("experts_down_scale"), dtype,
                                                f"layer {i} experts")
        if any(experts_i4):
            if not all(experts_i4):
                raise SamdError(f"a mix of INT4 and other sparse layers ({sum(experts_i4)} of {len(experts_i4)} carry INT4 experts): "
                                "the runner takes the experts of all sparse layers in one format")
            for i, l in enumerate(weights["layers"]):
                if "experts_gu" in l:
                    MOE.check_int4_experts((l["experts_gu"], l.get("experts_gu_z"), l.get("experts_gu_s")),
                                           (l["experts_down"], l.get("experts_down_z"), l.get("experts_down_s")), dtype, f"layer {i} experts")
        self.draft_head = bool(draft_head)
        require_gpu()
        self.shape, self.dtype, self.device = shape, dtype, torch.device(device)
        self.dt = torch_dtype_code(dtype)
        if self.dt not in (F16, BF16):
            raise SamdError("LlamaRunner computes in fp16 or bf16")
        self.weight_format = _weight_format(weight_format, weights, dtype)
        f8, f4, i4 = self.weight_format == "fp8", self.weight_format == "mxfp4", self.weight_format == "int4g128"
        quant = f8 or f4 or i4
        if f8 and not native_gemm:
            raise SamdError("FP8 projections exist only in the streaming kernel's packed form: native_gemm=False is not available with weight_format 'fp8'")
        if f4 and not native_gemm:
            raise SamdError("MXFP4 projections exist only in the streaming kernel's packed form: native_gemm=False is not available with weight_format 'mxfp4'")
        if i4 and not native_gemm:
            raise SamdError("INT4 projections exist only in the streaming kernel's packed form: native_gemm=False is not available with weight_format 'int4g128'")
        s = shape
        self.w = weights
        streams = lambda t: bool(native_gemm) and t.shape[0] % 128 == 0 and t.shape[1] % 256 == 0
        self.native_gemm_max_rows = int(os.environ.get("SAMD_NATIVE_GEMM_MAX_ROWS", 64))
        moe = shape.moe
        self.route_log = None
        if quant or moe:
            self.native_gemm_max_rows = TILE_ROWS
        self.layer_hook = None
        self.warm_kb = int(os.environ.get("SAMD_L2_WARM_KB", 0))
        self.warm_delay = int(os.environ.get("SAMD_L2_WARM_DELAY", 0))
        self.warm_where = int(os.environ.get("SAMD_L2_WARM_WHERE", 0))
        self.attention = attention or os.environ.get("SAMD_ATTENTION", "split")
        if self.attention not in ("split", "split2", "split3", "block"):
            raise SamdError(f"unknown attention mode '{self.attention}'")
        self.qkv_epilogue = bool(s.qkv_bias or s.qk_norm)
        if self.qkv_epilogue and self.attention not in ("split", "split3"):
            raise SamdError(f"attention mode '{self.attention}' rotates q / k inside its own kernel, which has no q|k|v bias or q / k norm: "
                            f"use 'split' or 'split3' for this model")
        self.v_layout_t = self.attention == "block" or (self.attention in ("split", "split3") and s.head_dim == 128
                                                        and os.environ.get("SAMD_V_LAYOUT", "t") != "rows")
        self.v_transposed = self.v_layout_t
        def pack(t):
            if not streams(t):
                return None
            out = torch.empty_like(t)
            check(lib().samd_gemm_pack_weights(_ptr(t), _ptr(out), t.shape[0], t.shape[1], current_stream()))
            return out
        def pack_gate_up(t):
            if s.inter % 16 != 0 or not streams(t):
                return None
            gate, up = t[:s.inter].view(s.inter // 16, 16, -1), t[s.inter:].view(s.inter // 16, 16, -1)
            w = torch.stack([gate, up], dim=1).reshape(2 * s.inter, -1).contiguous()
            out = torch.empty_like(w)
            check(lib().samd_gemm_pack_groups(_ptr(w), _ptr(out), 2 * s.inter, w.shape[1], current_stream()))
            return out
        def pack_qkv64(t):
            heads_total = s.heads + 2 * s.kv_heads
            mode = os.environ.get("SAMD_QKV_FUSED", "1")
            n_cols = heads_total * 128
            enough = n_cols // 64 >= 128 or (n_cols % 48 == 0 and n_cols // 48 >= 128)
            if (not streams(t) or self.attention != "split" or (not enough and mode != "force") or s.head_dim != 128 or mode == "0"
                    or self.qkv_epilogue):
                return None
            out = torch.empty_like(t)
            check(lib().samd_gemm_pack_qkv64(_ptr(t), _ptr(out), heads_total, t.shape[1], current_stream()))
            return out
        def pack_groups(t, fold):
            if not fold or t.shape[0] % 16 != 0 or t.shape[1] % 256 != 0:
                return None
            out = torch.empty_like(t)
            check(lib().samd_gemm_pack_groups(_ptr(t), _ptr(out), t.shape[0], t.shape[1], current_stream()))
            return out
        def pack_f8(l, k):
            t = l[k]
            N, K = t.shape
            if N % 128 != 0 or K % 256 != 0:
                raise SamdError(f"FP8 projection {k} of shape {tuple(t.shape)}: the FP8 kernel needs N % 128 == 0 and K % 256 == 0")
            if t.dtype == torch.float8_e4m3fn:
                q, scale = t.to(self.device).contiguous(), l.pop(k + "_scale").to(device=self.device, dtype=torch.float32).contiguous()
            else:
                q, scale = F8.quantize_rows(t)
            l[k] = torch.empty(t.shape, dtype=torch.float8_e4m3fn, device="meta")
            del t
            out = torch.empty_like(q)
            check(lib().samd_gemm_pack_f8(_ptr(q), _ptr(out), N, K, current_stream()))
            return out, scale
        def pack_f4(l, k):
            t = l[k]
            N, K = (t.shape[0], 2 * t.shape[1]) if _is_f4_tensor(t) else t.shape
            if N % 128 != 0 or K % 256 != 0:
                raise SamdError(f"MXFP4 projection {k} of shape ({N}, {K}): the MXFP4 kernel needs N % 128 == 0 and K % 256 == 0")
            if _is_f4_tensor(t):
                q, e8 = MX.fuse_mxfp4([(t, l.pop(k + "_e8"))], self.device)
                if tuple(e8.shape) != (N, K // 32):
                    raise SamdError(f"MXFP4 projection {k}: block scales of shape {tuple(e8.shape)} for a ({N}, {K}) matrix")
                MX.check_exponents(e8, dtype, f"MXFP4 projection {k}")
            else:
                q, e8 = MX.quantize_blocks(t, dtype)
            l[k] = torch.empty((N, K), dtype=torch.uint8, device="meta")
            del t
            out = torch.empty(MX.packed_bytes(N, K), dtype=torch.uint8, device=self.device)
            check(lib().samd_gemm_pack_f4(_ptr(q), _ptr(e8), _ptr(out), N, K, current_stream()))
            return out
        def pack_i4(l, k):
            t = l[k]
            if k + "_z" in l:
                q, z, sc = I4.fuse_int4([(t, l.pop(k + "_z"), l.pop(k + "_s"))], self.device, dtype)
            else:
                if t.shape[0] % 128 != 0 or t.shape[1] % 256 != 0:
                    raise SamdError(f"INT4 projection {k} of shape {tuple(t.shape)}: the INT4 kernel needs N % 128 == 0 and K % 256 == 0")
                q, z, sc = I4.quantize_groups(t, dtype)
            I4.check_groups(q, z, sc, dtype, k)
            N, K = q.shape[0], 2 * q.shape[1]
            l[k] = torch.empty((N, K), dtype=torch.uint8, device="meta")
            del t
            out = torch.empty(I4.packed_bytes(N, K), dtype=torch.uint8, device=self.device)
            check(lib().samd_gemm_pack_i4(_ptr(q), _ptr(z), _ptr(sc), _ptr(out), N, K, self.dt, current_stream()))
            return out
        layers = []
        for l in weights["layers"]:
            if i4:
                lp = dict(wqkv=None, wqkv64=None, wo=None, wo_g=None, wgu=None, wdown=None, wdown_g=None)
                for k in I4.PROJECTIONS:
                    lp[k + "_i4"] = pack_i4(l, k)
                layers.append(lp)
                continue
            if f4:
                lp = dict(wqkv=None, wqkv64=None, wo=None, wo_g=None, wgu=None, wdown=None, wdown_g=None)
                for k in MX.PROJECTIONS:
                    lp[k + "_f4"] = pack_f4(l, k)
                layers.append(lp)
                continue
            if f8:
                lp = dict(wqkv=None, wqkv64=None, wo=None, wo_g=None, wgu=None, wdown=None, wdown_g=None)
                for k in F8.PROJECTIONS:
                    lp[k + "_f8"] = pack_f8(l, k)
                layers.append(lp)
                continue
            sparse = "experts_gu" in l
            lp = dict(wgu=None if sparse else pack_gate_up(l["wgu"]), wqkv64=pack_qkv64(l["wqkv"]))
            lp["wqkv"] = pack(l["wqkv"]) if lp["wqkv64"] is None else None
            fold = (lp["wqkv64"] is not None and lp["wgu"] is not None and s.hidden <= 8192 and os.environ.get("SAMD_NORM_FOLD", "1") != "0"
                    and not moe)
            if sparse:
                gu_cols = s.hidden // 2 if MOE.is_4bit(l["experts_gu"]) else s.hidden
                if tuple(l["router"].shape) != (s.n_experts, s.hidden) or tuple(l["experts_gu"].shape) != (s.n_experts, 2 * s.moe_inter, gu_cols):
                    raise SamdError(f"sparse layer weights of shapes {tuple(l['router'].shape)}, {tuple(l['experts_gu'].shape)} do not match the shape")
                if self.expert_format == "mxfp4":
                    ekeys = ("experts_gu", "experts_gu_scale", "experts_down", "experts_down_scale")
                    if MOE.is_4bit(l["experts_gu"]):
                        quad = tuple(MX._bytes(l[k]).to(self.device).contiguous() for k in ekeys)
                    else:
                        quad = MOE.quantize_experts(l["experts_gu"], l["experts_down"], dtype, f"layer {len(layers)} experts")
                    lp["moe_gu"], lp["moe_down"] = MOE.pack_experts_mxfp4(*quad)
                    for k, t in zip(ekeys, quad):
                        l[k] = torch.empty(t.shape, dtype=torch.uint8, device="meta")
                    del quad
                elif self.expert_format == "int4g128":
                    gkeys, dkeys = ("experts_gu", "experts_gu_z", "experts_gu_s"), ("experts_down", "experts_down_z", "experts_down_s")
                    if "experts_gu_z" in l:
                        gu3, dn3 = (tuple(l[k].to(self.device).contiguous() for k in ks) for ks in (gkeys, dkeys))
                    else:
                        gu3, dn3 = MOE.quantize_experts_int4(l["experts_gu"], l["experts_down"], dtype, f"layer {len(layers)} experts")
                    lp["moe_gu"], lp["moe_down"] = MOE.pack_experts_int4(gu3, dn3, dtype)
                    for k, t in zip(gkeys + dkeys, gu3 + dn3):
                        l[k] = torch.empty(t.shape, dtype=t.dtype, device="meta")
                    del gu3, dn3
                else:
                    lp["moe_gu"], lp["moe_down"] = MOE.pack_experts(l["experts_gu"], l["experts_down"])
                    for k in ("experts_gu", "experts_down"):
                        l[k] = torch.empty(l[k].shape, dtype=l[k].dtype, device="meta")
                lp["wo_g"], lp["wdown_g"], lp["wdown"] = pack_groups(l["wo"], fold), None, None
                lp["wo"] = pack(l["wo"])
                layers.append(lp)
                continue
            lp["wo_g"], lp["wdown_g"] = pack_groups(l["wo"], fold), pack_groups(l["wdown"], fold)
            both = os.environ.get("SAMD_GEMM_ONE_COPY", "0") != "1"
            for k in ("wo", "wdown"):
                gm_ok = lp[k + "_g"] is not None and l[k].shape[0] % 128 == 0
                lp[k] = pack(l[k]) if (both or not gm_ok) else None
            layers.append(lp)
        self.wp = dict(lm_head=packed_lm_head if packed_lm_head is not None else pack(weights["lm_head"]), layers=layers)
        self.native_gemm = self.wp["lm_head"] is not None or any(v is not None for l in self.wp["layers"] for v in l.values())
        if not self.native_gemm:
            self.wp = None
        self.fused_mlp = self.wp is not None and all(l["wgu"] is not None for l in self.wp["layers"] if "moe_gu" not in l)
        self.norm_fold = (self.wp is not None and self.attention == "split"
                          and all(l.get("wo_g") is not None and l.get("wdown_g") is not None for l in self.wp["layers"]))
        self.scale = 1.0 / math.sqrt(s.head_dim)
        self.epi = self.epi_nobias = None
        if self.qkv_epilogue:
            def epi(l, bias):
                return QkvEpilogue(l["bqkv"].data_ptr() if bias and l.get("bqkv") is not None else None,
                                   l["q_norm"].data_ptr() if l.get("q_norm") is not None else None,
                                   l["k_norm"].data_ptr() if l.get("k_norm") is not None else None, s.eps)
            for l in weights["layers"]:
                if s.qkv_bias != (l.get("bqkv") is not None) or s.qk_norm != (l.get("q_norm") is not None and l.get("k_norm") is not None):
                    raise SamdError("the layer weights do not match the shape's qkv_bias / qk_norm")
                if s.qkv_bias and tuple(l["bqkv"].shape) != ((s.heads + 2 * s.kv_heads) * s.head_dim,):
                    raise SamdError(f"q|k|v bias of shape {tuple(l['bqkv'].shape)}")
                if s.qk_norm and (tuple(l["q_norm"].shape) != (s.head_dim,) or tuple(l["k_norm"].shape) != (s.head_dim,)):
                    raise SamdError("q_norm / k_norm weights must have head_dim elements")
                for k in ("bqkv", "q_norm", "k_norm"):
                    t = l.get(k)
                    if t is not None and (t.dtype != dtype or t.device.type != self.device.type or not t.is_contiguous()):
                        raise SamdError(f"{k} must be a contiguous {dtype} tensor on the GPU")
            self.epi = [epi(l, True) for l in weights["layers"]]
            self.epi_nobias = [epi(l, False) for l in weights["layers"]]
        self.row_major_released = quant or moe
        if moe and self.wp:
            for l, lp in zip(self.w["layers"], self.wp["layers"]):
                for k in ("wqkv", "wo", "wgu", "wdown"):
                    packed = lp.get(k) is not None or lp.get(k + "_g") is not None or (k == "wqkv" and lp.get("wqkv64") is not None)
                    if k in l and packed and l[k].device.type != "meta":
                        l[k] = torch.empty(l[k].shape, dtype=l[k].dtype, device="meta")
            torch.cuda.empty_cache()
        self._length_state(max_cache_len, kv)
        if os.environ.get("SAMD_RELEASE_ROW_MAJOR", "0") == "1":
            self.release_row_major()

    def memory_report(self):
        def nbytes(t):
            return 0 if t is None or t.device.type == "meta" else t.numel() * t.element_size()
        epi_keys = ("bqkv", "q_norm", "k_norm")
        rep = dict(row_major=sum(nbytes(t) for l in self.w["layers"] for k, t in l.items() if k not in epi_keys and k != "router")
                   + nbytes(self.w["lm_head"]) + nbytes(self.w["embed"]))
        if self.shape.moe:
            rep["moe_router"] = sum(nbytes(l.get("router")) for l in self.w["layers"])
            for k in ("moe_gu", "moe_down"):
                rep["packed_" + k] = sum(nbytes(l.get(k)) for l in (self.wp["layers"] if self.wp else ()))
        if self.qkv_epilogue:
            rep["qkv_epilogue"] = sum(nbytes(l.get(k)) for l in self.w["layers"] for k in epi_keys)
        if self.wp:
            for k in ("wqkv", "wqkv64", "wo", "wo_g", "wgu", "wdown", "wdown_g"):
                rep["packed_" + k] = sum(nbytes(l.get(k)) for l in self.wp["layers"])
            rep["packed_lm_head"] = nbytes(self.wp["lm_head"])
            if self.weight_format == "fp8":
                for k in F8.PROJECTIONS:
                    rep["packed_" + k + "_f8"] = sum(nbytes(l[k + "_f8"][0]) for l in self.wp["layers"])
                rep["fp8_scales"] = sum(nbytes(l[k + "_f8"][1]) for l in self.wp["layers"] for k in F8.PROJECTIONS)
            if self.weight_format == "mxfp4":
                for k in MX.PROJECTIONS:
                    rep["packed_" + k + "_f4"] = sum(nbytes(l[k + "_f4"]) * 16 // 17 for l in self.wp["layers"])
                rep["mxfp4_scales"] = sum(nbytes(l[k + "_f4"]) // 17 for l in self.wp["layers"] for k in MX.PROJECTIONS)
            if self.weight_format == "int4g128":
                for k in I4.PROJECTIONS:
                    rep["packed_" + k + "_i4"] = sum(nbytes(l[k + "_i4"]) * 16 // 17 for l in self.wp["layers"])
                rep["int4_group_data"] = sum(nbytes(l[k + "_i4"]) // 17 for l in self.wp["layers"] for k in I4.PROJECTIONS)
        rep["total"] = sum(rep.values())
        if self.weight_format in ("fp8", "mxfp4", "int4g128"):
            rep["weight_format"] = self.weight_format
        rep["expert_format"] = self.expert_format
        return rep

    def release_row_major(self):
        if self.row_major_released or not self.wp:
            return self.row_major_released
        if self.native_gemm_max_rows < TILE_ROWS:
            return False
        if self.wp["lm_head"] is None or any(l.get("wgu") is None or (l.get(k) is None and l.get(k + "_g") is None) for l in self.wp["layers"] for k in ("wo", "wdown")) or \
                any(l.get("wqkv") is None and l.get("wqkv64") is None for l in self.wp["layers"]):
            return False
        for l in self.w["layers"]:
            for k in ("wqkv", "wo", "wgu", "wdown"):
                l[k] = torch.empty(l[k].shape, dtype=l[k].dtype, device="meta")
        for lp in self.wp["layers"]:
            for k in ("wo", "wdown"):
                if lp.get(k) is not None and lp.get(k + "_g") is not None:
                    lp[k] = None
        self.row_major_released = True
        torch.cuda.empty_cache()
        return True

    def _length_state(self, max_cache_len, kv=None):
        s, dtype = self.shape, self.dtype
        self.max_len = int(max_cache_len)
        self.v_transposed = self.v_layout_t
        if self.v_transposed and (self.max_len < 8 or self.max_len % 8 != 0):
            if self.attention == "block":
                raise SamdError(f"max_cache_len {self.max_len} must be a multiple of 8 (16-byte loads along the transposed V cache)")
            self.v_transposed = False
# ... 179 lines not shown

    @classmethod
    def _hf_experts_are_4bit(cls, lyr, i):
        ex = lyr.mlp.experts
        gu, dn = MOE.is_4bit(ex.gate_up_proj), MOE.is_4bit(ex.down_proj)
        if gu != dn:
            raise SamdError(f"layers.{i}.mlp.experts: gate_up_proj is {ex.gate_up_proj.dtype} and down_proj {ex.down_proj.dtype}; "
                            "4-bit experts need both tensors 4-bit")
        return gu

    @classmethod
    def _hf_experts_are_int4(cls, lyr, i):
        ex = getattr(getattr(lyr, "mlp", None), "experts", None)
        if ex is None or hasattr(ex, "gate_up_proj") or not hasattr(ex, "__len__") or not hasattr(ex, "__getitem__"):
            return False
        kinds = [(f"layers.{i}.mlp.experts.{e}.{p}", I4.is_int4_module(getattr(ex[e], p, None)))
                 for e in range(len(ex)) for p in MOE.INT4_EXPERT_PROJECTIONS]
        n4 = sum(k for _, k in kinds)
        if 0 < n4 < len(kinds):
            plain = [n for n, k in kinds if not k][:3]
            raise SamdError(f"layers.{i}.mlp.experts: a mix of INT4 and other expert projections ({n4} of {len(kinds)} are INT4; e.g. "
                            f"{', '.join(plain)} are not): INT4 experts need gate_proj, up_proj and down_proj of every expert INT4")
        return n4 > 0

    _LAYER_PARAMS = ("self_attn.q_proj.weight", "self_attn.k_proj.weight", "self_attn.v_proj.weight", "self_attn.o_proj.weight",
                     "mlp.gate_proj.weight", "mlp.up_proj.weight", "mlp.down_proj.weight", "input_layernorm.weight", "post_attention_layernorm.weight")
    _QKV_BIAS = ("self_attn.q_proj.bias", "self_attn.k_proj.bias", "self_attn.v_proj.bias")
    _QK_NORM = ("self_attn.q_norm.weight", "self_attn.k_norm.weight")

    @classmethod
    def _hf_layer_extras(cls, layers):
        if len(layers) == 0:
            raise SamdError("the model has no decoder layers")
        def names_of(lyr, i):
            skip = {f"{n[:-len('.weight')]}.{sc}" for n, p in lyr.named_parameters()
                    if n.endswith(".weight") and (F8.is_fp8_dtype(p.dtype) or _is_f4_tensor(p))
                    for sc in ("weight_scale", "input_scale")}
            params = dict(lyr.named_parameters())
            for n, mod in lyr.named_modules():
                if n and I4.is_int4_module(mod):
                    for own in list(params):
                        if own.startswith(n + "."):
                            del params[own]
                    params[n + ".weight"] = None
                    if getattr(mod, "bias", None) is not None:
                        params[n + ".bias"] = None
            if any(MOE.is_4bit(params.get(n)) for n in MOE.SPARSE_MLP_PARAMS[1:]):
                skip |= set(MOE.EXPERT_SCALE_PARAMS)
            if cls._hf_experts_are_int4(lyr, i):
                for e in range(len(lyr.mlp.experts)):
                    for pn in MOE.INT4_EXPERT_PROJECTIONS:
                        params.pop(f"mlp.experts.{e}.{pn}.weight", None)
                params.update({n: None for n in MOE.SPARSE_MLP_PARAMS[1:]})
            return set(params) - skip
        names0 = names_of(layers[0], 0)
        qkv_bias = any(n in names0 for n in cls._QKV_BIAS)
        qk_norm = any(n in names0 for n in cls._QK_NORM)
        want = set(cls._LAYER_PARAMS) | (set(cls._QKV_BIAS) if qkv_bias else set()) | (set(cls._QK_NORM) if qk_norm else set())
        want_sparse = (want - set(MOE.DENSE_MLP_PARAMS)) | set(MOE.SPARSE_MLP_PARAMS)
        for i, lyr in enumerate(layers):
            names = names_of(lyr, i)
            if names == want:
                continue
            if any(n.startswith("mlp.experts.") or n == "mlp.gate.weight" for n in names):
                if names == want_sparse:
                    continue
                if any("shared_expert" in n for n in names):
                    raise SamdError(f"layer {i}: a shared expert is not supported (parameters {sorted(n for n in names if 'shared_expert' in n)})")
                raise SamdError(f"layer {i}: sparse MLP parameters the runner does not consume {sorted(names - want_sparse)}, or lacks "
                                f"{sorted(want_sparse - names)} (it reads mlp.gate.weight and the fused mlp.experts.gate_up_proj / down_proj)")
            extra, missing = sorted(names - want), sorted(want - names)
            if "self_attn.o_proj.bias" in extra:
                raise SamdError(f"layer {i}: o_proj bias is not supported (q|k|v biases are)")
            if any(n.startswith("mlp.") and n.endswith(".bias") for n in extra):
                raise SamdError(f"layer {i}: MLP projection biases are not supported")
            raise SamdError(f"layer {i}: parameters the runner does not consume {extra}, or lacks {missing} "
                            f"(it reads the Llama layer, q|k|v biases (Qwen2) and q / k norm weights (Qwen3))")
        return qkv_bias, qk_norm

    @classmethod
    def _hf_sparse_layers(cls, layers):
        return [any(n.startswith("mlp.experts.") for n, _ in lyr.named_parameters()) or cls._hf_experts_are_int4(lyr, i)
                for i, lyr in enumerate(layers)]

    @classmethod
    def random_init(cls, cfg, max_cache_len, dtype=torch.float16, device="cuda", seed=0, std=0.02, weight_format=None, expert_format=MOE.AUTO, **kw):
        require_gpu()
        shape = LlamaShape(cfg)
        MOE.resolve_expert_format(expert_format, False, shape.moe)
        g = torch.Generator(device=device).manual_seed(seed)

        def rnd(*size):
            return (torch.randn(size, generator=g, device=device, dtype=torch.float32) * std).to(dtype)
        s = shape
        qkv_out = (s.heads + 2 * s.kv_heads) * s.head_dim
        if s.moe:
            MOE.reject_unsupported(_env_weight_format(weight_format), kw.get("native_gemm", True), kw.get("draft_head", False))

        def mlp(i):
            if s.sparse[i]:
                return dict(router=rnd(s.n_experts, s.hidden), experts_gu=rnd(s.n_experts, 2 * s.moe_inter, s.hidden),
                            experts_down=rnd(s.n_experts, s.hidden, s.moe_inter))
            return dict(wgu=rnd(2 * s.inter, s.hidden), wdown=rnd(s.hidden, s.inter))
        layers = [dict(wqkv=rnd(qkv_out, s.hidden), wo=rnd(s.hidden, s.heads * s.head_dim), **mlp(i),
                       ln1=torch.ones(s.hidden, dtype=dtype, device=device),
                       ln2=torch.ones(s.hidden, dtype=dtype, device=device)) for i in range(s.layers)]

        def norm_w():
            mag = 0.5 + 1.5 * torch.rand(s.head_dim, generator=g, device=device)
            sign = torch.where(torch.rand(s.head_dim, generator=g, device=device) < 0.5, -1.0, 1.0)
            return (mag * sign).to(dtype)
        for l in layers:
            if s.qkv_bias:
                l["bqkv"] = (torch.randn(qkv_out, generator=g, device=device, dtype=torch.float32) * 0.5).to(dtype)
            if s.qk_norm:
                l["q_norm"], l["k_norm"] = norm_w(), norm_w()
        weights = dict(embed=rnd(s.vocab, s.hidden), layers=layers, norm=torch.ones(s.hidden, dtype=dtype, device=device),
                       lm_head=rnd(s.vocab, s.hidden))
        return cls(shape, weights, max_cache_len, dtype, device, weight_format=_env_weight_format(weight_format), expert_format=expert_format, **kw)

    def weight_bytes(self, experts=None):
        n_act = self.shape.top_k if experts is None else int(experts)
        nb = lambda t: t.numel() * t.element_size() if t.dim() != 3 else t[0].numel() * t.element_size() * min(n_act, t.shape[0])
        n = nb(self.w["lm_head"]) + nb(self.w["norm"])
        if self.weight_format in ("mxfp4", "int4g128"):
            sfx = "_f4" if self.weight_format == "mxfp4" else "_i4"
            for l, lp in zip(self.w["layers"], self.wp["layers"]):
                n += sum(nb(t) for k, t in l.items() if k not in MX.PROJECTIONS) + sum(nb(lp[k + sfx]) for k in MX.PROJECTIONS)
            return n
        for l in self.w["layers"]:
            n += sum(nb(t) for t in l.values())
        if self.weight_format == "fp8":
            n += sum(nb(l[k + "_f8"][1]) for l in self.wp["layers"] for k in F8.PROJECTIONS)
        return n

    def _rows_pad(self, R):
        return max(R, 16) if self.native_gemm else R

    def _buffers(self, R):
        if R not in self._buf:
            s, dt, dev = self.shape, self.dtype, self.device
            RP = self._rows_pad(R)
            z = lambda r, *sz: torch.zeros((max(r, RP),) + sz, dtype=dt, device=dev)
            ws_bytes = max(lib().samd_tree_attention_workspace(R, s.heads, s.head_dim), lib().samd_tree_attention_rope_workspace(R, s.heads, s.head_dim))
            part_elems = 0
            if self.native_gemm:
                qkv_out = (s.heads + 2 * s.kv_heads) * s.head_dim
                for n, k in ((qkv_out, s.hidden), (s.hidden, s.heads * s.head_dim), (2 * s.inter, s.hidden), (s.hidden, s.inter)):
                    if RP <= self.native_gemm_max_rows:
                        part_elems = max(part_elems, lib().samd_gemm_splits(n, k, RP) * RP * n)
            self._buf[R] = dict(x=z(R, s.hidden), h=z(R, s.hidden), qkv=z(R, (s.heads + 2 * s.kv_heads) * s.head_dim),
                                q=z(R, s.heads, s.head_dim), attn=z(R, s.heads, s.head_dim), o=z(R, s.hidden),
                                gu=z(R, 2 * s.inter), act=z(R, s.inter), d=z(R, s.hidden), logits=z(R, s.vocab),
                                argmax=torch.zeros(MAX_DRAFT, dtype=torch.int32, device=dev), rows_pad=RP,
                                part=torch.zeros(max(part_elems, 1), dtype=torch.float32, device=dev),
                                ws=torch.zeros(ws_bytes, dtype=torch.uint8, device=dev), ws_bytes=ws_bytes,
                                cs=torch.zeros((MAX_DRAFT, s.head_dim), dtype=torch.float32, device=dev),
                                ssq=torch.zeros((max(s.hidden // 16, 1), 16), dtype=torch.float32, device=dev))
            if s.moe:
                self._buf[R]["moe"] = MOE.MoeBuffers(RP, s.hidden, s.moe_inter, s.n_experts, s.top_k, dt, self.dt, dev)
        return self._buf[R]

    def max_draft_rows(self):
        wide_ok = (not self.row_major_released) and self.attention in ("split", "split3") and not getattr(self, "draft_head", False)
        return MAX_DRAFT if wide_ok else min(MAX_DRAFT, 64)

    def bucket(self, n):
        for b in self.BUCKETS:
            if n <= b:
                return b
        raise SamdError(f"draft of {n} nodes exceeds {MAX_DRAFT}")

    def forward_rows(self, R, d_tokens, d_relpos, d_mask, d_L, d_n, x_in=None, d_vis=None):
        if self.shape.moe:
            MOE.reject_unsupported(draft_head=getattr(self, "draft_head", False))
        if self._rows_pad(R) > self.native_gemm_max_rows and self.row_major_released:
            raise SamdError(f"a {R}-row forward needs the row-major projection matrices (released: SAMD_RELEASE_ROW_MAJOR / release_row_major()); "
                            f"drafts above {self.native_gemm_max_rows} nodes and the library-GEMM path are unavailable on this runner")
        L, s, b, dt, st = lib(), self.shape, self._buffers(R), self.dt, current_stream()
        RP, part = b["rows_pad"], b["part"]
        if (self.norm_fold and RP == 16 and x_in is None and d_vis is None and not getattr(self, "draft_head", False)
                and RP <= self.native_gemm_max_rows):
            return self._forward_rows_fold(R, b, d_tokens, d_relpos, d_mask, d_L, d_n)

        def hint(w, wp, fused=False, is_head=False):
            if wp is None or RP > self.native_gemm_max_rows or self.warm_kb <= 0:
                return None
            n, k = w.shape
            sp = 1 if (fused or is_head) else L.samd_gemm_splits(n, k, RP)
            return C.byref(Warm(wp.data_ptr(), n, k, sp, self.warm_kb, self.warm_delay, self.warm_where))

        def gemm(a, w, wp, out, wg=None, f8=None, f4=None, i4=None):
            n, k = w.shape
            if i4 is not None:
                sp = L.samd_gemm_splits(n, k, RP)
                check(L.samd_gemm_skinny_i4(_ptr(a), _ptr(i4), RP, n, k, sp, _ptr(part), _ptr(out), dt, st))
                return (out, 0, 0) if sp == 1 else (part, sp, RP * n)
            if f4 is not None:
                sp = L.samd_gemm_splits(n, k, RP)
                check(L.samd_gemm_skinny_f4(_ptr(a), _ptr(f4), RP, n, k, sp, _ptr(part), _ptr(out), dt, st))
                return (out, 0, 0) if sp == 1 else (part, sp, RP * n)
            if f8 is not None:
                sp = L.samd_gemm_splits(n, k, RP)
                check(L.samd_gemm_skinny_f8(_ptr(a), _ptr(f8[0]), _ptr(f8[1]), RP, n, k, sp, _ptr(part), _ptr(out), dt, st))
                return (out, 0, 0) if sp == 1 else (part, sp, RP * n)
            if (wp is None and wg is None) or RP > self.native_gemm_max_rows:
                torch.mm(a[:R], w.t(), out=out[:R])
                return out, 0, 0
            sp = L.samd_gemm_splits(n, k, RP) if out is not b["logits"] else 1
            if wp is not None and os.environ.get("SAMD_GEMM_PREFER_GROUPS", "0") != "1":
                check(L.samd_gemm_skinny(_ptr(a), _ptr(wp), RP, n, k, sp, _ptr(part), _ptr(out), dt, st))
            else:
                check(L.samd_gemm_skinny_groups(_ptr(a), _ptr(wg if wg is not None else wp), RP, n, k, sp, _ptr(part), _ptr(out), dt, st))
            return (out, 0, 0) if sp == 1 else (part, sp, RP * n)

        if x_in is None:
            check(L.samd_embed_rows(_ptr(d_tokens), _ptr(self.w["embed"]), _ptr(b["x"]), R, s.hidden, s.vocab, dt, st))
        else:
            rows_in = min(R, x_in.shape[0])
            if x_in.data_ptr() != b["x"].data_ptr():
                b["x"][:rows_in].copy_(x_in[:rows_in])
        head = getattr(self, "draft_head", False)
        log_routes = s.moe and self.route_log is not None and not torch.cuda.is_current_stream_capturing()
        block = self.attention == "block"
        vt = self.v_transposed and not block
        if self.attention != "split3":
            check(L.samd_rope_rows(_ptr(d_relpos), _ptr(d_vis if d_vis is not None else d_L), _ptr(self.cos), _ptr(self.sin), _ptr(b["cs"]), R,
                                   s.head_dim, self.rope_rows, st))
        if d_vis is not None and not block:
            raise SamdError("a visible length different from the write position needs attention mode 'block'")
        delta, dn, dstride = None, 0, 0
        packed = self.wp["layers"] if self.wp else [{}] * len(self.w["layers"])
        for li, w in enumerate(self.w["layers"]):
            if self.layer_hook is not None:
                self.layer_hook(li)
            wp = packed[li]
            raw_in = head and li == 0
            if not raw_in:
                check(L.samd_rmsnorm_warm(_ptr(b["x"]), _ptr(delta), _ptr(w["ln1"]), _ptr(b["h"]), R, s.hidden, s.eps, dt, dn, dstride,
                                          hint(w["wqkv"], wp.get("wqkv")), st))
            fused_qkv = wp.get("wqkv64") is not None and self.attention == "split" and RP <= self.native_gemm_max_rows and d_vis is None
            if fused_qkv:
                check((L.samd_gemm_qkv_rope_vt if vt else L.samd_gemm_qkv_rope)(
                    _ptr(b["x"] if raw_in else b["h"]), _ptr(wp["wqkv64"]), RP, s.hidden, _ptr(b["cs"]), _ptr(d_L), _ptr(d_n),
                    _ptr(b["q"]), _ptr(self.kv[li, 0]), _ptr(self.kv[li, 1]), s.heads, s.kv_heads, s.head_dim, self.max_len, dt, st))
            else:
                src, n_p, stride = gemm(b["x"] if raw_in else b["h"], w["wqkv"], wp.get("wqkv"), b["qkv"], f8=wp.get("wqkv_f8"), f4=wp.get("wqkv_f4"), i4=wp.get("wqkv_i4"))
            if block:
                check(L.samd_attention_block(_ptr(src), n_p, stride, _ptr(b["cs"]), _ptr(self.kv[li, 0]), _ptr(self.kv[li, 1]), _ptr(b["attn"]), dt, R,
                                             s.heads, s.kv_heads, s.head_dim, self.max_len, _ptr(d_mask), _ptr(d_L), _ptr(d_vis), _ptr(d_n), self.scale, st))
            elif self.attention == "split2":
                check(L.samd_tree_attention_rope(_ptr(src), n_p, stride, _ptr(b["cs"]), _ptr(self.kv[li, 0]), _ptr(self.kv[li, 1]), _ptr(b["attn"]), dt, R,
                                                 s.heads, s.kv_heads, s.head_dim, self.max_len, _ptr(d_mask), _ptr(d_L), _ptr(d_n), self.scale,
                                                 _ptr(b["ws"]), b["ws_bytes"], st))
            else:
                if fused_qkv:
                    pass
                elif self.epi is not None:
                    cs_form = self.attention == "split"
                    check(L.samd_rope_kv_write_epi(
                        _ptr(src), _ptr(d_relpos), _ptr(d_L), _ptr(d_n), None if cs_form else _ptr(self.cos), None if cs_form else _ptr(self.sin),
                        _ptr(b["cs"]) if cs_form else None, _ptr(b["q"]), _ptr(self.kv[li, 0]), _ptr(self.kv[li, 1]), int(vt), R, s.heads,
                        s.kv_heads, s.head_dim, self.max_len, self.rope_rows, dt, n_p, stride, C.byref(self.epi[li]), st))
                elif self.attention == "split":
                    check((L.samd_rope_kv_write_cs_vt if vt else L.samd_rope_kv_write_cs)(
                        _ptr(src), _ptr(d_relpos), _ptr(d_L), _ptr(d_n), _ptr(b["cs"]), _ptr(b["q"]), _ptr(self.kv[li, 0]),
                        _ptr(self.kv[li, 1]), R, s.heads, s.kv_heads, s.head_dim, self.max_len, dt, n_p, stride, st))
                else:
                    check((L.samd_rope_kv_write_vt if vt else L.samd_rope_kv_write)(
                        _ptr(src), _ptr(d_relpos), _ptr(d_L), _ptr(d_n), _ptr(self.cos), _ptr(self.sin),
                        _ptr(b["q"]), _ptr(self.kv[li, 0]), _ptr(self.kv[li, 1]), R, s.heads, s.kv_heads,
                        s.head_dim, self.max_len, self.rope_rows, dt, n_p, stride, st))
                check((L.samd_tree_attention_vt if vt else L.samd_tree_attention_warm)(
                    _ptr(b["q"]), _ptr(self.kv[li, 0]), _ptr(self.kv[li, 1]), _ptr(b["attn"]), dt, R, s.heads,
                    s.kv_heads, s.head_dim, self.max_len, _ptr(d_mask), _ptr(d_L), _ptr(d_n), self.scale,
                    _ptr(b["ws"]), b["ws_bytes"], hint(w["wo"], wp.get("wo")), st))
            src, n_p, stride = gemm(b["attn"].view(b["attn"].shape[0], -1), w["wo"], wp.get("wo"), b["o"], wg=wp.get("wo_g"), f8=wp.get("wo_f8"), f4=wp.get("wo_f4"), i4=wp.get("wo_i4"))
            check(L.samd_rmsnorm_warm(_ptr(b["x"]), _ptr(src), _ptr(w["ln2"]), _ptr(b["h"]), R, s.hidden, s.eps, dt, n_p, stride,
                                      None, st))
            if "moe_gu" in wp:
                mb = b["moe"]
                mb.route(b["h"], w["router"], d_n, s.norm_topk)
                if log_routes:
                    idx = mb.topk_idx.clone()
                    self.route_log.append((li, int((idx[:, 0] >= 0).sum()), idx, mb.topk_w.clone()))
                delta, dn, dstride = mb.experts(b["h"], wp["moe_gu"], wp["moe_down"], d_n, self.expert_format), 0, 0
                continue
            if wp.get("wgu") is not None and RP <= self.native_gemm_max_rows:
                check(L.samd_gemm_pairs_silu(_ptr(b["h"]), _ptr(wp["wgu"]), RP, s.inter, s.hidden, _ptr(b["act"]), dt, st))
            else:
                src, n_p, stride = gemm(b["h"], w["wgu"], None, b["gu"], f8=wp.get("wgu_f8"), f4=wp.get("wgu_f4"), i4=wp.get("wgu_i4"))
                check(L.samd_silu_mul(_ptr(src), _ptr(b["act"]), R, s.inter, dt, n_p, stride, st))
            delta, dn, dstride = gemm(b["act"], w["wdown"], wp.get("wdown"), b["d"], wg=wp.get("wdown_g"), f8=wp.get("wdown_f8"), f4=wp.get("wdown_f4"), i4=wp.get("wdown_i4"))
        check(L.samd_rmsnorm_warm(_ptr(b["x"]), _ptr(delta), _ptr(self.w["norm"]), _ptr(b["h"]), R, s.hidden, s.eps, dt, dn, dstride,
                                  hint(self.w["lm_head"], self.wp["lm_head"] if self.wp else None, is_head=True), st))
        gemm(b["x"] if head else b["h"], self.w["lm_head"], self.wp["lm_head"] if self.wp else None, b["logits"])
        if not head:
            check(L.samd_argmax_rows(_ptr(b["logits"]), dt, R, s.vocab, s.vocab, None, _ptr(b["argmax"]), st))
        return b

    def _forward_rows_fold(self, R, b, d_tokens, d_relpos, d_mask, d_L, d_n):
        L, s, dt, st = lib(), self.shape, self.dt, current_stream()
        x, ssq = b["x"], b["ssq"]
        rows_cs = 8 if R <= 8 else 16
        rows_a = rows_cs if os.environ.get("SAMD_NORM_ROWS8", "1") != "0" else 16
        if s.head_dim == 128 and os.environ.get("SAMD_FUSE_EMBED_ROPE", "1") != "0":
            check(L.samd_embed_rows_ssq_rope(_ptr(d_tokens), _ptr(self.w["embed"]), _ptr(x), _ptr(ssq), 16, s.hidden, s.vocab, dt, _ptr(d_relpos), _ptr(d_L),
                                             _ptr(self.cos), _ptr(self.sin), _ptr(b["cs"]), R, s.head_dim, self.rope_rows, st))
        else:
            check(L.samd_embed_rows_ssq(_ptr(d_tokens), _ptr(self.w["embed"]), _ptr(x), _ptr(ssq), 16, s.hidden, s.vocab, dt, st))
            check(L.samd_rope_rows(_ptr(d_relpos), _ptr(d_L), _ptr(self.cos), _ptr(self.sin), _ptr(b["cs"]), R, s.head_dim, self.rope_rows, st))
        attn2d = b["attn"].view(b["attn"].shape[0], -1)
        qkv_launch = L.samd_gemm_qkv_rope_norm_vt if self.v_transposed else L.samd_gemm_qkv_rope_norm
        attn_launch = L.samd_tree_attention_vt if self.v_transposed else L.samd_tree_attention_warm
        for li, (w, wp) in enumerate(zip(self.w["layers"], self.wp["layers"])):
            if self.layer_hook is not None:
                self.layer_hook(li)
            check(qkv_launch(_ptr(x), _ptr(ssq), _ptr(w["ln1"]), s.eps, _ptr(wp["wqkv64"]), rows_a, s.hidden, _ptr(b["cs"]), _ptr(d_L), _ptr(d_n),
                             _ptr(b["q"]), _ptr(self.kv[li, 0]), _ptr(self.kv[li, 1]), s.heads, s.kv_heads, s.head_dim, self.max_len, dt, st))
            check(attn_launch(_ptr(b["q"]), _ptr(self.kv[li, 0]), _ptr(self.kv[li, 1]), _ptr(b["attn"]), dt, R, s.heads,
                              s.kv_heads, s.head_dim, self.max_len, _ptr(d_mask), _ptr(d_L), _ptr(d_n), self.scale,
                              _ptr(b["ws"]), b["ws_bytes"], None, st))
            check(L.samd_gemm_cs_residual(_ptr(attn2d), _ptr(wp["wo_g"]), rows_cs, s.hidden, attn2d.shape[1], _ptr(x), _ptr(ssq), dt, st))
            check(L.samd_gemm_pairs_silu_norm(_ptr(x), _ptr(ssq), _ptr(w["ln2"]), s.eps, _ptr(wp["wgu"]), rows_a, s.inter, s.hidden, _ptr(b["act"]), dt, st))
            check(L.samd_gemm_cs_residual(_ptr(b["act"]), _ptr(wp["wdown_g"]), rows_cs, s.hidden, s.inter, _ptr(x), _ptr(ssq), dt, st))
        check(L.samd_rmsnorm(_ptr(x), None, _ptr(self.w["norm"]), _ptr(b["h"]), R, s.hidden, s.eps, dt, 0, 0, st))
        wl = self.wp["lm_head"]
        if wl is not None:
            check(L.samd_gemm_skinny(_ptr(b["h"]), _ptr(wl), 16, s.vocab, s.hidden, 1, _ptr(b["part"]), _ptr(b["logits"]), dt, st))
        else:
            torch.mm(b["h"][:R], self.w["lm_head"].t(), out=b["logits"][:R])
        check(L.samd_argmax_rows(_ptr(b["logits"]), dt, R, s.vocab, s.vocab, None, _ptr(b["argmax"]), st))
        return b

    def prefill(self, session: Session, input_ids, on_chunk=None):
        ids = input_ids.reshape(-1).to(device=self.device, dtype=torch.int32)
        N = ids.numel()
        if N < 1 or N > self.max_len:
            raise SamdError(f"prompt of {N} tokens does not fit max_cache_len {self.max_len}")
        if N >= 2 * TILE_ROWS and os.environ.get("SAMD_PREFILL", "wide") != "chunked" and not self.row_major_released:
            return self._prefill_wide(session, ids, on_chunk)
        v = session.device_views()
        b = None
        for c0 in range(0, N, TILE_ROWS):
            n = min(TILE_ROWS, N - c0)
            self.pf_tokens.zero_()
            self.pf_tokens[:n] = ids[c0:c0 + n]
            self.pf_n.fill_(n)
            session.set_cache_length(c0)
            b = self.forward_rows(TILE_ROWS, self.pf_tokens, self.pf_relpos, self.pf_mask, v["cache_length"], self.pf_n)
            if on_chunk is not None:
                on_chunk(self.pf_tokens, b["logits"], n, b["h"])
        session.set_cache_length(N)
        session.set_start_token(b["argmax"][(N - 1) % TILE_ROWS:])
        return b["logits"][(N - 1) % TILE_ROWS]

    PF_SPLIT_MIN_ROWS = 1024
    PF_ATTN_PAD = 128

    def _is_gfx950(self):
        if not hasattr(self, "_gfx950"):
            name = getattr(torch.cuda.get_device_properties(self.device), "gcnArchName", "") or ""
            self._gfx950 = name.split(":")[0] == "gfx950"
        return self._gfx950

    def _time_mm(self, x, wt, out, reps=3):
        best = float("inf")
        torch.mm(x, wt, out=out)
        for _ in range(reps):
            e0, e1 = torch.cuda.Event(enable_timing=True), torch.cuda.Event(enable_timing=True)
            e0.record()
            torch.mm(x, wt, out=out)
            e1.record()
            e1.synchronize()
            best = min(best, e0.elapsed_time(e1))
        return best

    def tune_prefill(self, max_rows=None):
        self._pf_plan = {}
        if os.environ.get("SAMD_PREFILL_SPLIT", "1") == "0" or self.row_major_released:
            return self._pf_plan
        max_rows = min(int(max_rows or self.max_len), 4096)
        w0 = self.w["layers"][0]
        try:
            for key in ("wqkv", "wo", "wgu", "wdown"):
                wt = w0[key].t()
                K, N = wt.shape
                x = torch.zeros((max_rows + 64, K), dtype=self.dtype, device=self.device)
                out = torch.empty((max_rows + 64, N), dtype=self.dtype, device=self.device)
                small = {r: self._time_mm(x[:r], wt, out[:r]) for r in (64, 128, 192, 256)}
                plan = {}
                for R in range(max(256, (self.PF_SPLIT_MIN_ROWS // 256) * 256), max_rows, 256):
                    t_at = self._time_mm(x[:R], wt, out[:R])
                    t_past = self._time_mm(x[:R + 64], wt, out[:R + 64])
                    plan[R] = {r: t_at + small[r] < 0.95 * t_past for r in small}
                self._pf_plan[key] = plan
                del x, out
        except RuntimeError as e:
            import warnings
            warnings.warn(f"tune_prefill: measurement failed ({str(e)[:120]}); projections of long prompts stay single library calls", RuntimeWarning)
            self._pf_plan = {}
        return self._pf_plan

    def prefill_plan_summary(self):
        plan = getattr(self, "_pf_plan", None) or {}
        return {k: [R for R, d in sorted(v.items()) if any(d.values())] for k, v in plan.items()}

    def _pf_split(self, key, M):
        if M <= self.PF_SPLIT_MIN_ROWS:
            return 0
        if getattr(self, "_pf_plan", None) is None:
            self.tune_prefill()
        R = ((M - 1) // 256) * 256
        rest = -(-(M - R) // 64) * 64
        return R if self._pf_plan.get(key, {}).get(R, {}).get(rest, False) else 0

    def _pf_mm(self, x, w, out, key, bias=None):
        R = self._pf_split(key, x.shape[0])
        mm = torch.mm if bias is None else (lambda a, b, out: torch.addmm(bias, a, b, out=out))
        if R:
            mm(x[:R], w.t(), out=out[:R])
            mm(x[R:], w.t(), out=out[R:])
        else:
            mm(x, w.t(), out=out)

    def _prefill_wide(self, session: Session, ids, on_chunk=None):
        L, s, dt, st, N = lib(), self.shape, self.dt, current_stream(), ids.numel()
        dev, ty = self.device, self.dtype
        z = lambda *sz: torch.empty(sz, dtype=ty, device=dev)
        x, h = z(N, s.hidden), z(N, s.hidden)
        own_attn = (s.head_dim == 128 and os.environ.get("SAMD_PREFILL_ATTENTION", "own") != "sdpa"
                    and self._is_gfx950())
        Np = N if own_attn else -(-N // self.PF_ATTN_PAD) * self.PF_ATTN_PAD
        if Np > self.max_len:
            Np = N
        ao = z(N, s.heads * s.head_dim) if own_attn else None
        qkv_p, qp = z(Np, (s.heads + 2 * s.kv_heads) * s.head_dim), z(Np, s.heads, s.head_dim)
        qkv, q = qkv_p[:N], qp[:N]
        if Np > N:
            qp[N:].zero_()
            if self.v_transposed:
                qkv_p[N:].zero_()
                self.kv[:, 0, :, N:Np].zero_()
            else:
                self.kv[:, :, :, N:Np].zero_()
        o, gu, act, d = z(N, s.hidden), z(N, 2 * s.inter), z(N, s.inter), z(N, s.hidden)
        relpos = torch.arange(N, dtype=torch.int32, device=dev)
        d_L = torch.zeros(1, dtype=torch.int32, device=dev)
        d_n = torch.full((1,), N, dtype=torch.int32, device=dev)
        check(L.samd_embed_rows(_ptr(ids), _ptr(self.w["embed"]), _ptr(x), N, s.hidden, s.vocab, dt, st))
        delta = None
        for li, w in enumerate(self.w["layers"]):
            check(L.samd_rmsnorm(_ptr(x), _ptr(delta), _ptr(w["ln1"]), _ptr(h), N, s.hidden, s.eps, dt, 0, 0, st))
            self._pf_mm(h, w["wqkv"], qkv, "wqkv", bias=w.get("bqkv"))
            if self.epi is not None:
                check(L.samd_rope_kv_write_epi(_ptr(qkv), _ptr(relpos), _ptr(d_L), _ptr(d_n), _ptr(self.cos), _ptr(self.sin), None, _ptr(q),
                                               _ptr(self.kv[li, 0]), _ptr(self.kv[li, 1]), int(self.v_transposed), N, s.heads, s.kv_heads,
                                               s.head_dim, self.max_len, self.rope_rows, dt, 0, 0, C.byref(self.epi_nobias[li]), st))
                if self.v_transposed:
                    vv = qkv_p[:, (s.heads + s.kv_heads) * s.head_dim:].view(Np, s.kv_heads, s.head_dim).transpose(0, 1)
                else:
                    vv = self.kv[li, 1][:, :Np]
            elif self.v_transposed:
                check(L.samd_rope_kv_write_vt(_ptr(qkv), _ptr(relpos), _ptr(d_L), _ptr(d_n), _ptr(self.cos), _ptr(self.sin), _ptr(q),
                                              _ptr(self.kv[li, 0]), _ptr(self.kv[li, 1]), N, s.heads, s.kv_heads, s.head_dim, self.max_len,
                                              self.rope_rows, dt, 0, 0, st))
                vv = qkv_p[:, (s.heads + s.kv_heads) * s.head_dim:].view(Np, s.kv_heads, s.head_dim).transpose(0, 1)
            else:
                check(L.samd_rope_kv_write(_ptr(qkv), _ptr(relpos), _ptr(d_L), _ptr(d_n), _ptr(self.cos), _ptr(self.sin), _ptr(q),
                                           _ptr(self.kv[li, 0]), _ptr(self.kv[li, 1]), N, s.heads, s.kv_heads, s.head_dim, self.max_len,
                                           self.rope_rows, dt, 0, 0, st))
                vv = self.kv[li, 1][:, :Np]
            if own_attn:
                check((L.samd_prefill_attention_vt if self.v_transposed else L.samd_prefill_attention)(
                    _ptr(q), _ptr(self.kv[li, 0]), _ptr(self.kv[li, 1]), _ptr(ao), dt, N, 0, s.heads, s.kv_heads,
                    s.head_dim, self.max_len, self.scale, st))
                self._pf_mm(ao, w["wo"], o, "wo")
            else:
                kk = self.kv[li, 0][:, :Np]
                if s.kv_heads != s.heads:
                    kk, vv = kk.repeat_interleave(s.heads // s.kv_heads, dim=0), vv.repeat_interleave(s.heads // s.kv_heads, dim=0)
                att = torch.nn.functional.scaled_dot_product_attention(qp.transpose(0, 1)[None], kk[None], vv[None], is_causal=True, scale=self.scale)
                self._pf_mm(att[0, :, :N].transpose(0, 1).reshape(N, -1), w["wo"], o, "wo")
            check(L.samd_rmsnorm(_ptr(x), _ptr(o), _ptr(w["ln2"]), _ptr(h), N, s.hidden, s.eps, dt, 0, 0, st))
            self._pf_mm(h, w["wgu"], gu, "wgu")
            check(L.samd_silu_mul(_ptr(gu), _ptr(act), N, s.inter, dt, 0, 0, st))
            self._pf_mm(act, w["wdown"], d, "wdown")
            delta = d
        check(L.samd_rmsnorm(_ptr(x), _ptr(delta), _ptr(self.w["norm"]), _ptr(h), N, s.hidden, s.eps, dt, 0, 0, st))
        b = self._buffers(1)
        if on_chunk is None:
            torch.mm(h[N - 1:N], self.w["lm_head"].t(), out=b["logits"][:1])
        else:
            logits = torch.mm(h, self.w["lm_head"].t())
            for c0 in range(0, N, TILE_ROWS):
                n = min(TILE_ROWS, N - c0)
                on_chunk(ids[c0:c0 + n], logits[c0:c0 + n], n, h[c0:c0 + n])
            b["logits"][:1].copy_(logits[N - 1:N])
        check(L.samd_argmax_rows(_ptr(b["logits"]), dt, 1, s.vocab, s.vocab, None, _ptr(b["argmax"]), st))
        session.set_cache_length(N)
        session.set_start_token(b["argmax"])
        return b["logits"][0]

    def warm(self, R):
        self.pf_n.zero_()
        scratch_L = torch.zeros(1, dtype=torch.int32, device=self.device)
        self.forward_rows(R, self.pf_tokens, self.pf_relpos, self.pf_mask, scratch_L, self.pf_n)
        torch.cuda.current_stream().synchronize()

    def hidden_rows(self, R):
        return self._buffers(R)["h"]

    def forward_tokens(self, session: Session, tokens, relpos, mask_rows, n, L, return_hidden=False):
        R = self.bucket(n)
        tok = torch.zeros(MAX_DRAFT, dtype=torch.int32, device=self.device)
        tok[:n] = tokens.reshape(-1)[:n].to(torch.int32)
        rel = torch.zeros(MAX_DRAFT, dtype=torch.int32, device=self.device)
        rel[:n] = relpos.reshape(-1)[:n].to(torch.int32)
        d_n = torch.tensor([n], dtype=torch.int32, device=self.device)
        session.set_cache_length(L)
        b = self.forward_rows(R, tok, rel, mask_rows, session.device_views()["cache_length"], d_n)
        torch.cuda.current_stream().synchronize()
        return (b["logits"][:n], b["h"][:n]) if return_hidden else b["logits"][:n]

    def verify(self, session: Session, R):
        v = session.device_views()
        n_ptr = C.c_void_p(v["dmeta"] + 4)
        return self.forward_rows(R, v["tokens"], v["position"], v["mask"], v["cache_length"], n_ptr)

    def compact(self, session: Session):
        s = self.shape
        session.kv_compact(self.kv_ptrs, 2 * s.layers, s.kv_heads, self.max_len, s.head_dim, self.kv.element_size(), n_transposed=s.layers if self.v_transposed else 0)
```

Baseline: 814.5.

## Add 6/10-row fold buckets and stage norm weights once in LDS

Adds finer row buckets (6, 8, 10, 16) to the norm-fold GEMM kernels and the runner, so short verify batches stage fewer activation rows and fewer waves do staging work. The RMSNorm gain vector is now loaded once per block into extra LDS and read from there, instead of being reloaded from global memory for every K chunk in the pipelined loop. This reduces global load traffic and vmcnt pressure. In exchange it uses more LDS per block and adds more template instantiations and bucket graphs.

```diff
diff --git a/sam-decoding_amd/csrc/gemm_kernels.hip b/sam-decoding_amd/csrc/gemm_kernels.hip
--- a/sam-decoding_amd/csrc/gemm_kernels.hip
+++ b/sam-decoding_amd/csrc/gemm_kernels.hip
@@ -202,6 +202,30 @@
     asm volatile("" ::: "memory");
 }
 
+#define NORM_GR 2
+template <int NT>
+__device__ __forceinline__ void norm_g_issue(const NormArgs &na, int units , u32x4 (&gv)[NORM_GR]) {
+    const int tid = threadIdx.x;
+#pragma unroll
+    for (int k = 0; k < NORM_GR; k++) {
+        gv[k] = (u32x4){0u, 0u, 0u, 0u};
+        if (NT * k >= units) continue;
+        int u = tid + NT * k;
+        u = u < units ? u : units - 1;
+        const u32x4 *src = reinterpret_cast<const u32x4 *>(na.g) + u;
+        asm volatile("global_load_dwordx4 %0, %1, off" : "=v"(gv[k]) : "v"(src) : "memory");
+    }
+}
+template <int NT>
+__device__ __forceinline__ void norm_g_store(int units, u32x4 (&gv)[NORM_GR], u32x4 *gl ) {
+    const int tid = threadIdx.x;
+    static_assert(NORM_GR == 2, "");
+    asm volatile("" : "+v"(gv[0]), "+v"(gv[1]) : : "memory");
+#pragma unroll
+    for (int k = 0; k < NORM_GR; k++)
+        if (tid + NT * k < units) gl[tid + NT * k] = gv[k];
+}
+
 template <typename E>
 __device__ __forceinline__ u32x4 norm_scale8(u32x4 xraw, u32x4 graw, float rs) {
     const E *xe = reinterpret_cast<const E *>(&xraw);
@@ -245,8 +269,8 @@
 
     const int tid = threadIdx.x, w = tid >> 6, l = tid & 63, n = l & 15, g = l >> 4;
     const bool streams = CG == 4 || w < 2 * CG;
-    static_assert(AR == 16 || (AR == 8 && NORM && RT == 1), "8 activation rows: the norm-fold kernels only");
-    const bool stager = AR == 16 || w < GEMM_WAVES / 2;
+    static_assert(AR == 16 || ((AR == 6 || AR == 8 || AR == 10) && NORM && RT == 1), "fewer than 16 activation rows: the norm-fold kernels only");
+    const bool stager = AR == 16 || w < AR / 2;
     const int cg = CG == 4 ? (w & 3) : (streams ? w % CG : 0), kh = CG == 4 ? (w >> 2) : (streams ? w / CG : 0);
     const char *wtile = reinterpret_cast<const char *>(W) + (size_t)blockIdx.x * n_chunks * CH;
     const uint32_t wlane = (uint32_t)(64 * (CG * kh + cg) + l) * 16;
@@ -265,16 +289,15 @@
             asm volatile("global_load_dwordx4 %0, %1, %2 nt" : "=v"(dst[bl][j]) : "v"(wlane), "s"(p + (CH / 4) * (2 * bl + j)) : "memory");
     };
     static_assert(!NORM || RT == 1, "the norm-fold path is built for the 16-row tile");
-    constexpr int XL = NORM ? 2 * XV : XV;
-    u32x4 xr[NORM ? DEPTH : 1][NORM ? XV : 1], gr[NORM ? DEPTH : 1][NORM ? XV : 1];
+    constexpr int XL = XV;
+    u32x4 xr[NORM ? DEPTH : 1][NORM ? XV : 1];
     __shared__ float norm_part[NORM ? (NT / 16) * 16 : 1], norm_rs[NORM ? 16 : 1];
+    u32x4 *gl = reinterpret_cast<u32x4 *>(gemm_lds + (size_t)NB * R * GEMM_KC * 2);
     auto stage_xi = [&](int c, int buf, int i, int d) {
         const int slot = tid + NT * i, row = slot >> 5, pos = slot & 31, unit = pos ^ (row & 15);
         const E *src = A + (size_t)row * K + (size_t)c * GEMM_KC + 8 * unit;
         if constexpr (NORM) {
-            const E *gsrc = reinterpret_cast<const E *>(na.g) + (size_t)c * GEMM_KC + 8 * unit;
             asm volatile("global_load_dwordx4 %0, %1, off" : "=v"(xr[d][i]) : "v"(src) : "memory");
-            asm volatile("global_load_dwordx4 %0, %1, off" : "=v"(gr[d][i]) : "v"(gsrc) : "memory");
         } else {
             E *dst = &xs[buf][0][0] + (size_t)(NT * i + 64 * w) * 8;
             __builtin_amdgcn_global_load_lds((gptr_t)src, (lptr_t)dst, 16, 0, 0);
@@ -288,27 +311,27 @@
             for (int i = 0; i < XV; i++) stage_xi(c, buf, i, d);
         }
     };
-    auto scale_to_lds = [&](int buf, int d) {
+    auto scale_to_lds = [&](int c, int buf, int d) {
         if constexpr (NORM) {
             if (!stager) return;
 #pragma unroll
             for (int i = 0; i < XV; i++) {
-                const int slot = tid + NT * i, row = slot >> 5;
-                asm volatile("" : "+v"(xr[d][i]), "+v"(gr[d][i]) : : "memory");
-                const u32x4 v = norm_scale8<E>(xr[d][i], gr[d][i], norm_rs[row]);
+                const int slot = tid + NT * i, row = slot >> 5, pos = slot & 31, unit = pos ^ (row & 15);
+                asm volatile("" : "+v"(xr[d][i]) : : "memory");
+                const u32x4 v = norm_scale8<E>(xr[d][i], gl[c * (GEMM_KC / 8) + unit], norm_rs[row]);
                 *reinterpret_cast<u32x4 *>(&xs[buf][0][0] + (size_t)slot * 8) = v;
             }
         }
     };
-    auto landed = [&](int younger, int buf, int d) {
+    auto landed = [&](int c, int younger, int buf, int d) {
         if (streams) { if (stager) gemm_wait_younger<DEPTH, WL + XL>(younger); else gemm_wait_younger<DEPTH, WL>(younger); }
         else { if (stager) gemm_wait_younger<DEPTH, XL>(younger); else gemm_wait_younger<DEPTH, 0>(younger); }
-        if constexpr (NORM) { scale_to_lds(buf, d); asm volatile("s_waitcnt lgkmcnt(0)" ::: "memory"); }
+        if constexpr (NORM) { scale_to_lds(c, buf, d); asm volatile("s_waitcnt lgkmcnt(0)" ::: "memory"); }
         __builtin_amdgcn_s_barrier();
         asm volatile("" ::: "memory");
     };
     auto phase = [&](u32x4 (&cur)[2][2], int c, int buf, int d) {
-        landed(n_chunks - 1 - c, buf, d);
+        landed(c, n_chunks - 1 - c, buf, d);
         const uint32_t xbase = lds_base + (uint32_t)buf * (R * GEMM_KC * 2) + (uint32_t)n * (GEMM_KC * 2);
 #pragma unroll
         for (int bl = 0; bl < 2; bl++) {
@@ -340,11 +363,12 @@
         if (c + DEPTH < n_chunks) issue(cur, c + DEPTH, buf == 0 ? NB - 1 : buf - 1, d);
     };
     float norm_sv[NORM ? NORM_NS : 1];
-    if constexpr (NORM) norm_issue<NT>(na, norm_sv);
+    u32x4 norm_gv[NORM ? NORM_GR : 1];
+    if constexpr (NORM) { norm_issue<NT>(na, norm_sv); norm_g_issue<NT>(na, K / 8, norm_gv); }
 #pragma unroll
     for (int d = 0; d < DEPTH; d++)
         if (d < n_chunks) issue(wr[d], d, d, d);
-    if constexpr (AR == 8) {
+    if constexpr (AR < 16) {
         if (!stager) {
 #pragma unroll
             for (int bz = 0; bz < NB; bz++) *reinterpret_cast<u32x4 *>(&xs[bz][0][0] + (size_t)tid * 8) = (u32x4){0u, 0u, 0u, 0u};
@@ -355,6 +379,7 @@
             if (streams) { if (stager) asm volatile("s_waitcnt vmcnt(%0)" : : "n"(DEPTH * (WL + XL)) : "memory"); else asm volatile("s_waitcnt vmcnt(%0)" : : "n"(DEPTH * WL) : "memory"); }
             else { if (stager) asm volatile("s_waitcnt vmcnt(%0)" : : "n"(DEPTH * XL) : "memory"); else asm volatile("s_waitcnt vmcnt(0)" : : : "memory"); }
         } else asm volatile("s_waitcnt vmcnt(0)" : : : "memory");
+        norm_g_store<NT>(K / 8, norm_gv, gl);
         norm_finish<NT>(na, norm_sv, norm_part, norm_rs);
     }
     {
@@ -443,8 +468,8 @@
 #endif
     const int p0 = (int)((long long)blockIdx.x * n_pairs / gridDim.x), p1 = (int)((long long)(blockIdx.x + 1) * n_pairs / gridDim.x);
     const bool active = w < 2 * (p1 - p0);
-    static_assert(AR == 16 || (AR == 8 && NORM && RT == 1), "8 activation rows: the norm-fold kernels only");
-    const bool stager = AR == 16 || w < GEMM_WAVES / 2;
+    static_assert(AR == 16 || ((AR == 6 || AR == 8 || AR == 10) && NORM && RT == 1), "fewer than 16 activation rows: the norm-fold kernels only");
+    const bool stager = AR == 16 || w < AR / 2;
     const int gi = 2 * p0 + w;
     const char *wgrp = reinterpret_cast<const char *>(W) + (size_t)(active ? gi : 0) * n_chunks * 8192;
     const uint32_t wlane = (uint32_t)l * 16;
@@ -463,9 +488,10 @@
                 asm volatile("global_load_dwordx4 %0, %1, %2 nt" : "=v"(dst[b][j]) : "v"(wlane), "s"(p + 1024 * (2 * b + j)) : "memory");
     };
     static_assert(!NORM || RT == 1, "the norm-fold path is built for the 16-row tile");
-    constexpr int XL = NORM ? 2 * XV : XV;
-    u32x4 xr[NORM ? DEPTH : 1][NORM ? XV : 1], gr[NORM ? DEPTH : 1][NORM ? XV : 1];
+    constexpr int XL = XV;
+    u32x4 xr[NORM ? DEPTH : 1][NORM ? XV : 1];
     __shared__ float norm_part[NORM ? (NT / 16) * 16 : 1], norm_rs[NORM ? 16 : 1];
+    u32x4 *gl = reinterpret_cast<u32x4 *>(gemm_lds + (size_t)NB * R * GEMM_KC * 2);
     auto stage_x = [&](int c, int buf, int d) {
         if (!stager || (abl & 4)) return;
 #pragma unroll
@@ -473,9 +499,7 @@
             const int slot = tid + NT * i, row = slot >> 5, pos = slot & 31, unit = pos ^ (row & 15);
             const E *src = A + (size_t)((abl & 8) ? (row & 15) : row) * K + (size_t)c * GEMM_KC + 8 * unit;
             if constexpr (NORM) {
-                const E *gsrc = reinterpret_cast<const E *>(na.g) + (size_t)c * GEMM_KC + 8 * unit;
                 asm volatile("global_load_dwordx4 %0, %1, off" : "=v"(xr[d][i]) : "v"(src) : "memory");
-                asm volatile("global_load_dwordx4 %0, %1, off" : "=v"(gr[d][i]) : "v"(gsrc) : "memory");
             } else {
                 E *dst = &xs[buf][0][0] + (size_t)(NT * i + 64 * w) * 8;
                 __builtin_amdgcn_global_load_lds((gptr_t)src, (lptr_t)dst, 16, 0, 0);
@@ -483,7 +507,7 @@
             }
         }
     };
-    auto landed = [&](int younger, int buf, int d) {
+    auto landed = [&](int c, int younger, int buf, int d) {
         const bool stg = stager && !(abl & 4);
         if (active) { if (stg) gemm_wait_younger<DEPTH, 8 + XL>(younger); else gemm_wait_younger<DEPTH, 8>(younger); }
         else { if (stg) gemm_wait_younger<DEPTH, XL>(younger); else gemm_wait_younger<DEPTH, 0>(younger); }
@@ -491,9 +515,9 @@
             if (stager) {
 #pragma unroll
                 for (int i = 0; i < XV; i++) {
-                    const int slot = tid + NT * i, row = slot >> 5;
-                    asm volatile("" : "+v"(xr[d][i]), "+v"(gr[d][i]) : : "memory");
-                    const u32x4 v = norm_scale8<E>(xr[d][i], gr[d][i], norm_rs[row]);
+                    const int slot = tid + NT * i, row = slot >> 5, pos = slot & 31, unit = pos ^ (row & 15);
+                    asm volatile("" : "+v"(xr[d][i]) : : "memory");
+                    const u32x4 v = norm_scale8<E>(xr[d][i], gl[c * (GEMM_KC / 8) + unit], norm_rs[row]);
                     *reinterpret_cast<u32x4 *>(&xs[buf][0][0] + (size_t)slot * 8) = v;
                 }
             }
@@ -503,7 +527,7 @@
         asm volatile("" ::: "memory");
     };
     auto phase = [&](u32x4 (&cur)[4][2], int c, int buf, int d) {
-        landed(n_chunks - 1 - c, buf, d);
+        landed(c, n_chunks - 1 - c, buf, d);
         if (active && !(abl & 2)) {
             const uint32_t xbase = lds_base + (uint32_t)buf * (R * GEMM_KC * 2) + (uint32_t)n * (GEMM_KC * 2);
 #pragma unroll
@@ -535,11 +559,12 @@
         if (c + DEPTH < n_chunks) { if (active) load_w(cur, c + DEPTH); stage_x(c + DEPTH, buf == 0 ? NB - 1 : buf - 1, d); }
     };
     float norm_sv[NORM ? NORM_NS : 1];
-    if constexpr (NORM) norm_issue<NT>(na, norm_sv);
+    u32x4 norm_gv[NORM ? NORM_GR : 1];
+    if constexpr (NORM) { norm_issue<NT>(na, norm_sv); norm_g_issue<NT>(na, K / 8, norm_gv); }
 #pragma unroll
     for (int d = 0; d < DEPTH; d++)
         if (d < n_chunks) { if (active) load_w(wr[d], d); stage_x(d, d, d); }
-    if constexpr (AR == 8) {
+    if constexpr (AR < 16) {
         if (!stager) {
 #pragma unroll
             for (int bz = 0; bz < NB; bz++) *reinterpret_cast<u32x4 *>(&xs[bz][0][0] + (size_t)tid * 8) = (u32x4){0u, 0u, 0u, 0u};
@@ -550,6 +575,7 @@
             if (active) { if (stager) asm volatile("s_waitcnt vmcnt(%0)" : : "n"(DEPTH * (8 + XL)) : "memory"); else asm volatile("s_waitcnt vmcnt(%0)" : : "n"(DEPTH * 8) : "memory"); }
             else { if (stager) asm volatile("s_waitcnt vmcnt(%0)" : : "n"(DEPTH * XL) : "memory"); else asm volatile("s_waitcnt vmcnt(0)" : : : "memory"); }
         } else asm volatile("s_waitcnt vmcnt(0)" : : : "memory");
+        norm_g_store<NT>(K / 8, norm_gv, gl);
         norm_finish<NT>(na, norm_sv, norm_part, norm_rs);
     }
     {
@@ -598,13 +624,13 @@
     const char *wgrp = reinterpret_cast<const char *>(W) + (size_t)blockIdx.x * n_chunks * 8192;
     const uint32_t wlane = (uint32_t)l * 16;
 
-    static_assert(ROWS == 8 || ROWS == 16, "");
+    static_assert(ROWS == 6 || ROWS == 8 || ROWS == 10 || ROWS == 16, "");
     constexpr int AL = ROWS / 2;
-    if constexpr (ROWS == 8) {
+    if constexpr (ROWS < 16) {
 #pragma unroll
         for (int buf = 0; buf < CSD; buf++)
 #pragma unroll
-            for (int i = 4; i < 8; i++)
+            for (int i = AL; i < 8; i++)
                 *reinterpret_cast<u32x4 *>(xs + (size_t)buf * 16 * GEMM_KC + (size_t)(64 * i + l) * 8) = (u32x4){0u, 0u, 0u, 0u};
         asm volatile("s_waitcnt lgkmcnt(0)" ::: "memory");
     }
@@ -745,8 +771,10 @@
 template <typename TT, int RT, int DEPTH, int CG, bool NORM = false, int AR = 16>
 static hipError_t qkv_rope_launch(hipStream_t st, const void *A, const void *W, int K, int tiles, const float *cs, const int *d_L, const int *d_n, void *q, void *k, void *v,
                                   int H, int Hkv, long long max_len, int v_t, NormArgs na = NormArgs{nullptr, nullptr, 0, 0.f, 0.f}) {
-    constexpr int lds_a = (DEPTH + 1) * 16 * RT * GEMM_KC * 2, lds_e = 2 * 16 * RT * 16 * CG * 4, lds = lds_a > lds_e ? lds_a : lds_e;
-    if constexpr (lds > 60000) {
+    constexpr int lds_a = (DEPTH + 1) * 16 * RT * GEMM_KC * 2, lds_e = 2 * 16 * RT * 16 * CG * 4, lds_s = lds_a > lds_e ? lds_a : lds_e;
+    static_assert(!NORM || lds_a + 8192 * 2 + 4096 <= 65536, "A buffers + the norm weights of K <= 8192 + the static arrays fit the default LDS limit");
+    const int lds = lds_s + (NORM ? K * 2 : 0);
+    if constexpr (lds_s > 60000) {
         static unsigned long long done = 0ull;
         const hipError_t attr = samd_reserve_lds((const void *)k_gemm_qkv_rope<TT, RT, DEPTH, CG, NORM, AR>, lds + 4096, &done);
         if (attr != hipSuccess) return attr;
@@ -759,8 +787,10 @@
 template <typename TT, int RT, int DEPTH, bool NORM = false, int AR = 16>
 static hipError_t pairs_silu_launch(hipStream_t st, int grid, const void *A, const void *W, void *out, int K, int inter, int n_pairs,
                                     NormArgs na = NormArgs{nullptr, nullptr, 0, 0.f, 0.f}) {
-    constexpr int lds_a = (DEPTH + 1) * 16 * RT * GEMM_KC * 2, lds_e = 4 * 16 * RT * 16 * 4, lds = lds_a > lds_e ? lds_a : lds_e;
-    if constexpr (lds > 60000) {
+    constexpr int lds_a = (DEPTH + 1) * 16 * RT * GEMM_KC * 2, lds_e = 4 * 16 * RT * 16 * 4, lds_s = lds_a > lds_e ? lds_a : lds_e;
+    static_assert(!NORM || lds_a + 8192 * 2 + 4096 <= 65536, "A buffers + the norm weights of K <= 8192 + the static arrays fit the default LDS limit");
+    const int lds = lds_s + (NORM ? K * 2 : 0);
+    if constexpr (lds_s > 60000) {
         static unsigned long long done = 0ull;
         const hipError_t attr = samd_reserve_lds((const void *)k_gemm_pairs_silu<TT, RT, DEPTH, NORM, AR>, lds + 4096, &done);
         if (attr != hipSuccess) return attr;
@@ -769,6 +799,8 @@
                        (typename TT::elem *)out, K, inter, K / GEMM_KC, n_pairs, na);
     return hipSuccess;
 }
+
+static bool fold_rows_ok(int rows_pad) { return rows_pad == 6 || rows_pad == 8 || rows_pad == 10 || rows_pad == 16; }
 
 extern "C" {
 
@@ -819,9 +851,9 @@
 
 int samd_gemm_pairs_silu_norm(const void *d_x, const float *d_ssq, const void *d_norm_weight, float eps, const void *d_Wg, int32_t rows_pad, int32_t inter, int32_t K,
                               void *d_out, int32_t dtype, void *stream) {
-    if (!d_x || !d_ssq || !d_norm_weight || !d_Wg || !d_out || (rows_pad != 16 && rows_pad != 8) || inter < 16 || inter % 16 != 0 || K < GEMM_KC || K % GEMM_KC != 0 ||
+    if (!d_x || !d_ssq || !d_norm_weight || !d_Wg || !d_out || !fold_rows_ok(rows_pad) || inter < 16 || inter % 16 != 0 || K < GEMM_KC || K % GEMM_KC != 0 ||
         K / 16 > 32 * NORM_NS || (dtype != SAMD_F16 && dtype != SAMD_BF16)) {
-        samd_set_error("samd_gemm_pairs_silu_norm: unsupported shape (8 or 16 rows, inter %% 16 == 0, K %% 256 == 0, K <= 8192, f16/bf16) or null pointer"); return SAMD_E_INVALID;
+        samd_set_error("samd_gemm_pairs_silu_norm: unsupported shape (6, 8, 10 or 16 rows, inter %% 16 == 0, K %% 256 == 0, K <= 8192, f16/bf16) or null pointer"); return SAMD_E_INVALID;
     }
     const int n_cu = samd_cu_count();
     const int n_pairs = inter / 16;
@@ -829,19 +861,19 @@
     while ((n_pairs + grid - 1) / grid > 4) grid += n_cu;
     const NormArgs na{d_ssq, d_norm_weight, K / 16, 1.f / (float)K, eps};
     hipStream_t st = (hipStream_t)stream;
-    const hipError_t e = rows_pad == 8
-        ? (dtype == SAMD_F16 ? pairs_silu_launch<GF16, 1, 3, true, 8>(st, grid, d_x, d_Wg, d_out, K, inter, n_pairs, na)
-                             : pairs_silu_launch<GBF16, 1, 3, true, 8>(st, grid, d_x, d_Wg, d_out, K, inter, n_pairs, na))
-        : (dtype == SAMD_F16 ? pairs_silu_launch<GF16, 1, 3, true>(st, grid, d_x, d_Wg, d_out, K, inter, n_pairs, na)
-                             : pairs_silu_launch<GBF16, 1, 3, true>(st, grid, d_x, d_Wg, d_out, K, inter, n_pairs, na));
+#define GO(TT, AR) pairs_silu_launch<TT, 1, 3, true, AR>(st, grid, d_x, d_Wg, d_out, K, inter, n_pairs, na)
+#define ROWS_GO(TT) (rows_pad == 6 ? GO(TT, 6) : rows_pad == 8 ? GO(TT, 8) : rows_pad == 10 ? GO(TT, 10) : GO(TT, 16))
+    const hipError_t e = dtype == SAMD_F16 ? ROWS_GO(GF16) : ROWS_GO(GBF16);
+#undef ROWS_GO
+#undef GO
     if (e != hipSuccess) { samd_set_error("samd_gemm_pairs_silu_norm: %s", hipGetErrorString(e)); return SAMD_E_HIP; }
     LAUNCHCHK();
     return SAMD_OK;
 }
 
 int samd_gemm_cs_residual(const void *d_A, const void *d_Wg, int32_t rows_pad, int32_t N, int32_t K, void *d_x, float *d_ssq, int32_t dtype, void *stream) {
-    if (!d_A || !d_Wg || !d_x || !d_ssq || (rows_pad != 16 && rows_pad != 8) || N < 16 || N % 16 != 0 || K < GEMM_KC || K % GEMM_KC != 0 || (dtype != SAMD_F16 && dtype != SAMD_BF16)) {
-        samd_set_error("samd_gemm_cs_residual: unsupported shape (8 or 16 rows, N %% 16 == 0, K %% 256 == 0, f16/bf16) or null pointer"); return SAMD_E_INVALID;
+    if (!d_A || !d_Wg || !d_x || !d_ssq || !fold_rows_ok(rows_pad) || N < 16 || N % 16 != 0 || K < GEMM_KC || K % GEMM_KC != 0 || (dtype != SAMD_F16 && dtype != SAMD_BF16)) {
+        samd_set_error("samd_gemm_cs_residual: unsupported shape (6, 8, 10 or 16 rows, N %% 16 == 0, K %% 256 == 0, f16/bf16) or null pointer"); return SAMD_E_INVALID;
     }
     constexpr int lds = GEMM_WAVES * 2 * 16 * GEMM_KC * 2;
     hipStream_t st = (hipStream_t)stream;
@@ -849,8 +881,9 @@
 #define GO(TT, ROWS, ET) do { static unsigned long long done = 0ull; \
         e = samd_reserve_lds((const void *)k_gemm_cs_residual<TT, ROWS>, lds, &done); \
         if (e == hipSuccess) hipLaunchKernelGGL((k_gemm_cs_residual<TT, ROWS>), dim3(N / 16), dim3(64 * GEMM_WAVES), lds, st, (const ET *)d_A, (const ET *)d_Wg, (ET *)d_x, d_ssq, K, N, K / GEMM_KC, (const int *)nullptr, (int *)nullptr, 0); } while (0)
-    if (dtype == SAMD_F16) { if (rows_pad == 8) GO(GF16, 8, _Float16); else GO(GF16, 16, _Float16); }
-    else { if (rows_pad == 8) GO(GBF16, 8, __bf16); else GO(GBF16, 16, __bf16); }
+#define ROWS_GO(TT, ET) do { if (rows_pad == 6) GO(TT, 6, ET); else if (rows_pad == 8) GO(TT, 8, ET); else if (rows_pad == 10) GO(TT, 10, ET); else GO(TT, 16, ET); } while (0)
+    if (dtype == SAMD_F16) ROWS_GO(GF16, _Float16); else ROWS_GO(GBF16, __bf16);
+#undef ROWS_GO
 #undef GO
     if (e != hipSuccess) { samd_set_error("samd_gemm_cs_residual: %s", hipGetErrorString(e)); return SAMD_E_HIP; }
     LAUNCHCHK();
@@ -964,8 +997,8 @@
                                    const float *d_cs, const int32_t *d_cache_length, const int32_t *d_n, void *d_q_out, void *d_k_cache, void *d_v_cache,
                                    int32_t n_heads, int32_t n_kv_heads, int32_t head_dim, int64_t max_len, int32_t dtype, void *stream, int v_t) {
     if (!d_x || !d_ssq || !d_norm_weight || !d_W64 || !d_cs || !d_cache_length || !d_n || !d_q_out || !d_k_cache || !d_v_cache || head_dim != 128 || n_heads < 1 ||
-        n_kv_heads < 1 || (rows_pad != 16 && rows_pad != 8) || K < GEMM_KC || K % GEMM_KC != 0 || K / 16 > 32 * NORM_NS || (dtype != SAMD_F16 && dtype != SAMD_BF16)) {
-        samd_set_error("samd_gemm_qkv_rope_norm: unsupported shape (8 or 16 rows, head_dim 128, K %% 256 == 0, K <= 8192, f16/bf16) or null pointer"); return SAMD_E_INVALID;
+        n_kv_heads < 1 || !fold_rows_ok(rows_pad) || K < GEMM_KC || K % GEMM_KC != 0 || K / 16 > 32 * NORM_NS || (dtype != SAMD_F16 && dtype != SAMD_BF16)) {
+        samd_set_error("samd_gemm_qkv_rope_norm: unsupported shape (6, 8, 10 or 16 rows, head_dim 128, K %% 256 == 0, K <= 8192, f16/bf16) or null pointer"); return SAMD_E_INVALID;
     }
     const int groups = qkv_tile_groups(n_heads + 2 * n_kv_heads);
     const int tiles = (n_heads + 2 * n_kv_heads) * 128 / (16 * groups);
@@ -973,13 +1006,10 @@
     hipStream_t st = (hipStream_t)stream;
     hipError_t e = hipSuccess;
 #define GO(TT, CG, AR) e = qkv_rope_launch<TT, 1, 4, CG, true, AR>(st, d_x, d_W64, K, tiles, d_cs, d_cache_length, d_n, d_q_out, d_k_cache, d_v_cache, n_heads, n_kv_heads, (long long)max_len, v_t, na)
-    if (rows_pad == 8) {
-        if (groups == 3) { if (dtype == SAMD_F16) GO(GF16, 3, 8); else GO(GBF16, 3, 8); }
-        else { if (dtype == SAMD_F16) GO(GF16, 4, 8); else GO(GBF16, 4, 8); }
-    } else {
-        if (groups == 3) { if (dtype == SAMD_F16) GO(GF16, 3, 16); else GO(GBF16, 3, 16); }
-        else { if (dtype == SAMD_F16) GO(GF16, 4, 16); else GO(GBF16, 4, 16); }
-    }
+#define ROWS_GO(TT, CG) do { if (rows_pad == 6) GO(TT, CG, 6); else if (rows_pad == 8) GO(TT, CG, 8); else if (rows_pad == 10) GO(TT, CG, 10); else GO(TT, CG, 16); } while (0)
+    if (groups == 3) { if (dtype == SAMD_F16) ROWS_GO(GF16, 3); else ROWS_GO(GBF16, 3); }
+    else { if (dtype == SAMD_F16) ROWS_GO(GF16, 4); else ROWS_GO(GBF16, 4); }
+#undef ROWS_GO
 #undef GO
     if (e != hipSuccess) { samd_set_error("samd_gemm_qkv_rope_norm: %s", hipGetErrorString(e)); return SAMD_E_HIP; }
     LAUNCHCHK();
diff --git a/sam-decoding_amd/samd_hip/llama.py b/sam-decoding_amd/samd_hip/llama.py
--- a/sam-decoding_amd/samd_hip/llama.py
+++ b/sam-decoding_amd/samd_hip/llama.py
@@ -118,7 +118,7 @@
 
 class LlamaRunner:
 
-    BUCKETS = (1, 8, 16, 32, 48, 64, 128)
+    BUCKETS = (1, 6, 8, 10, 16, 32, 48, 64, 128)
 
     def __init__(self, shape, weights, max_cache_len, dtype=torch.float16, device="cuda", kv=None, native_gemm=True, packed_lm_head=None,
                  attention=None, weight_format=None, draft_head=False, expert_format=MOE.AUTO):
@@ -904,7 +904,7 @@
     def _forward_rows_fold(self, R, b, d_tokens, d_relpos, d_mask, d_L, d_n):
         L, s, dt, st = lib(), self.shape, self.dt, current_stream()
         x, ssq = b["x"], b["ssq"]
-        rows_cs = 8 if R <= 8 else 16
+        rows_cs = next(r for r in (6, 8, 10, 16) if R <= r)
         rows_a = rows_cs if os.environ.get("SAMD_NORM_ROWS8", "1") != "0" else 16
         if s.head_dim == 128 and os.environ.get("SAMD_FUSE_EMBED_ROPE", "1") != "0":
             check(L.samd_embed_rows_ssq_rope(_ptr(d_tokens), _ptr(self.w["embed"]), _ptr(x), _ptr(ssq), 16, s.hidden, s.vocab, dt, _ptr(d_relpos), _ptr(d_L),
```

New measurement: 820.5 (median of 6 runs). Within noise of the previous version (+0.7%).
